# catid/video_stabilizer

Measured on AMD Instinct MI355X. Metric: aligned frames/sec, higher is better.
Workload: dtype u8

## Files before the change

include/vs_amd.h:

```cpp
#ifndef VS_AMD_H
#define VS_AMD_H

#include <stddef.h>
#include <stdint.h>

#ifdef __cplusplus
extern "C" {
#endif

#define VS_OK 0
#define VS_ERR_ARG (-1)
#define VS_ERR_HIP (-2)
#define VS_ERR_UNSUPPORTED (-3)
#define VS_ERR_STATE (-4)
#define VS_ERR_NOMEM (-5)

enum { VS_MEM_HOST = 0, VS_MEM_DEVICE = 1 };
enum { VS_FMT_GRAY8 = 0, VS_FMT_BGR8 = 1, VS_FMT_BGR10 = 2, VS_FMT_BGR12 = 3, VS_FMT_BGR16_FULL = 4 };
int vs_format_bits(int format);
int vs_format_max_value(int format);
enum { VS_WARP_LANCZOS2 = 0, VS_WARP_BILINEAR = 1, VS_WARP_LANCZOS2_FAST = 2, VS_WARP_LANCZOS2_SEP = 3, VS_WARP_BILINEAR_CV = 4 };
enum { VS_BORDER_CLAMP = 0, VS_BORDER_CONSTANT = 1 };
enum {
    VS_SELECT_STL_HOST = 0,
// ... 90 lines not shown
                            void* dst, size_t dst_frame_stride, int dst_stride, int mem, void* stream);
int vs_bgr_image_warp_roi_batch(const void* src, size_t src_frame_stride, int n_frames, int w, int h, int src_stride,
                                int channels, int bits, const vs_transform* t, int mode, int border, int max_value,
                                int roi_x, int roi_y, int roi_w, int roi_h,
                                void* dst, size_t dst_frame_stride, int dst_stride, int mem, void* stream);
int vs_bgr_image_warp_fill_batch(const void* src, size_t src_frame_stride, int n_src, int w, int h, int src_stride,
                                 int channels, int bits, int n_out, int n_cand, const int32_t* cand_frame,
                                 const vs_transform* cand_t, int border, int max_value,
                                 int roi_x, int roi_y, int roi_w, int roi_h,
                                 void* dst, size_t dst_frame_stride, int dst_stride, int mem, void* stream);
typedef struct vs_deblur_params { float sensitivity; float max_ratio; } vs_deblur_params;
void vs_deblur_params_default(vs_deblur_params* p);
int vs_bgr_sharpness_batch(const void* src, size_t src_frame_stride, int n, int w, int h, int src_stride, int format,
                           uint64_t* sharpness, int mem, void* stream);
int vs_bgr_deblur_batch(const void* src, size_t src_frame_stride, int n_src, int w, int h, int src_stride, int format,
                        const uint64_t* sharpness, int n_out, int n_cand, const int32_t* cand_frame, const vs_transform* cand_t,
                        const vs_deblur_params* params ,
                        void* dst, size_t dst_frame_stride, int dst_stride, int mem, void* stream);
int vs_bgr_image_warp_f32(const void* src, int w, int h, int src_stride, int channels, int bits,
                          const vs_transform* t, int mode, int border,
                          float* dst, int dst_stride, int mem, void* stream);
int vs_bgr_to_gray(const void* src, int w, int h, int src_stride, int bits, int shift_to_8,
                   uint8_t* dst, int dst_stride, int mem, void* stream);

typedef struct vs_flow_params {
    double pyr_scale;
    int    levels;
    int    winsize;
    int    iterations;
    int    poly_n;
    double poly_sigma;
    int    flags;
} vs_flow_params;
void vs_flow_params_default(vs_flow_params* p);
typedef struct vs_flow vs_flow;
vs_flow* vs_flow_create(const vs_flow_params* params , int device);
void     vs_flow_destroy(vs_flow* f);
int vs_flow_compute(vs_flow* f, const uint8_t* prev, const uint8_t* next, int w, int h, int stride, int mem, float* flow,
                    int flow_stride);
int vs_flow_jitter(vs_flow* f, const void* frames, size_t frame_stride, int n, int w, int h, int stride, int format, int mem,
                   float* pair_medians, double* median);

int vs_test_fail_alloc(int k);

int vs_debug_bounds_check(void);
int vs_debug_bounds_selftest(void);

int vs_calib_copy12(const void* src_dev, void* dst_dev, size_t bytes, void* stream);
int vs_shader_clock_probe(void* stream, double* shader_mhz);

typedef struct vs_aligner vs_aligner;
typedef struct vs_align_info {
    int32_t status;
    int32_t fail_reason;
    int32_t fail_level;
    int32_t levels;
    int32_t iterations[16];
    double  condition[16];
    double  phase_dx, phase_dy, phase_response;
    int32_t selected_x[16], selected_y[16];
    vs_transform level_transform[16];
} vs_align_info;

vs_aligner* vs_aligner_create(const vs_aligner_params* params , int device);
void vs_aligner_destroy(vs_aligner* a);
int  vs_aligner_set_select_mode(vs_aligner* a, int select_mode);
int  vs_aligner_get_select_mode(const vs_aligner* a);
enum { VS_BATCH_EXCLUSIVE = 0, VS_BATCH_SHARED = 1 };
int  vs_aligner_set_batch_mode(vs_aligner* a, int batch_mode);
int  vs_aligner_reset(vs_aligner* a);
void* vs_aligner_stream(const vs_aligner* a);
int   vs_aligner_wait_stream(vs_aligner* a, void* producer_stream);
int  vs_aligner_align_next(vs_aligner* a, const void* frame, int w, int h, int stride, int format, int mem,
                           const vs_aligner_params* params, vs_transform* out);
int  vs_aligner_align_batch(vs_aligner* a, const void* frames, size_t frame_stride, int n,
                            int w, int h, int stride, int format, int mem,
                            const vs_aligner_params* params, vs_transform* out, int32_t* status);
int  vs_aligner_align_clips(vs_aligner* a, const void* frames, size_t frame_stride, int n_clips, int frames_per_clip,
                            int w, int h, int stride, int format, int mem,
                            const vs_aligner_params* params, vs_transform* out, int32_t* status);
int  vs_aligner_get_info(const vs_aligner* a, int i, vs_align_info* info);
int  vs_aligner_level_dims(const vs_aligner* a, int level, int* w, int* h, int* tiles_x, int* tiles_y, int* tile_size);
int  vs_aligner_read_level_image(const vs_aligner* a, int i, int level, uint8_t* out);
int  vs_aligner_read_level_argmax(const vs_aligner* a, int i, int level, int set, uint16_t* out);
int  vs_aligner_read_level_jacobian(const vs_aligner* a, int i, int level, int set, float* out);

enum {
    VS_STAGE_INGEST = 0,
    VS_STAGE_PYR_DOWN = 1,
    VS_STAGE_KEYFRAME = 2,
    VS_STAGE_WARPDIFF = 3,
    VS_STAGE_SELECT = 4,
    VS_STAGE_GATHER = 5,
    VS_STAGE_GN = 6,
    VS_STAGE_PHASE = 7,
    VS_STAGE_COUNT = 8
};
typedef struct vs_stage_timings {
    double ms[VS_STAGE_COUNT];
    int64_t launches[VS_STAGE_COUNT];
    int64_t frames;
    int64_t gn_iterations;
} vs_stage_timings;
int  vs_aligner_enable_timing(vs_aligner* a, int enable);
int  vs_aligner_get_timings(vs_aligner* a, vs_stage_timings* out);

typedef struct vs_stabilizer vs_stabilizer;
vs_stabilizer* vs_stabilizer_create(const vs_stabilizer_params* params , int device);
void vs_stabilizer_destroy(vs_stabilizer* s);
int  vs_stabilizer_process(vs_stabilizer* s, const void* frame, int w, int h, int stride, int format, int mem,
                           void* out, int* out_w, int* out_h);
int  vs_stabilizer_process_batch(vs_stabilizer* s, const void* frames, size_t frame_stride, int n, int w, int h, int stride,
                                 int format, int mem, void* out, size_t out_frame_stride, int32_t* has_output,
                                 int* out_w, int* out_h);
int  vs_stabilizer_process_clips(vs_stabilizer* s, const void* frames, size_t frame_stride, int n_clips, int frames_per_clip,
                                 int w, int h, int stride, int format, int mem, void* out, size_t out_frame_stride,
                                 int32_t* has_output, int* out_w, int* out_h);
int  vs_stabilizer_reset(vs_stabilizer* s);
void* vs_stabilizer_stream(const vs_stabilizer* s);
int   vs_stabilizer_wait_stream(vs_stabilizer* s, void* producer_stream);
int   vs_stabilizer_set_select_mode(vs_stabilizer* s, int mode);
int   vs_stabilizer_get_select_mode(const vs_stabilizer* s);
int   vs_stabilizer_set_border_fill(vs_stabilizer* s, int ahead);
int   vs_stabilizer_get_border_fill(const vs_stabilizer* s);
int   vs_stabilizer_set_deblur(vs_stabilizer* s, int ahead, const vs_deblur_params* params);
int   vs_stabilizer_get_deblur(const vs_stabilizer* s);
void vs_stabilizer_state(const vs_stabilizer* s, vs_transform* last_meas, vs_transform* accum, int* last_success);

#ifdef __cplusplus
}
#endif
#endif
```

video_stabilizer_amd/capi.py:

```python
import ctypes as C
import os

import numpy as np

_HERE = os.path.dirname(os.path.abspath(__file__))
LIB_PATH = os.environ.get("VS_AMD_LIB", os.path.join(_HERE, "libvs_amd.so"))

MEM_HOST, MEM_DEVICE = 0, 1
FMT_GRAY8, FMT_BGR8 = 0, 1
FMT_BGR10, FMT_BGR12, FMT_BGR16_FULL = 2, 3, 4
WARP_LANCZOS2, WARP_BILINEAR, WARP_LANCZOS2_FAST, WARP_LANCZOS2_SEP, WARP_BILINEAR_CV = 0, 1, 2, 3, 4
BORDER_CLAMP, BORDER_CONSTANT = 0, 1
SELECT_STL_HOST, SELECT_DEVICE, SELECT_STABLE = 0, 1, 2
BATCH_EXCLUSIVE, BATCH_SHARED = 0, 1
ABI_VERSION = 5


class Transform(C.Structure):
    _fields_ = [("A", C.c_double), ("B", C.c_double), ("TX", C.c_double), ("TY", C.c_double)]

    def tup(self):
        return (self.A, self.B, self.TX, self.TY)

    @staticmethod
# ... 55 lines not shown

SIGNATURES = {
    "vs_last_error": (C.c_char_p, []),
    "vs_version": (C.c_char_p, []),
    "vs_abi_version": (_i32, []),
    "vs_sizeof_align_info": (_sz, []),
    "vs_test_fail_alloc": (_i32, [_i32]),
    "vs_debug_bounds_check": (_i32, []),
    "vs_debug_bounds_selftest": (_i32, []),
    "vs_device_count": (_i32, []),
    "vs_shader_clock_probe": (_i32, [C.c_void_p, C.POINTER(C.c_double)]),
    "vs_stream_retire": (_i32, [_vp]),
    "vs_format_bits": (_i32, [_i32]),
    "vs_format_max_value": (_i32, [_i32]),
    "vs_aligner_stream": (_vp, [_vp]),
    "vs_aligner_wait_stream": (_i32, [_vp, _vp]),
    "vs_stabilizer_stream": (_vp, [_vp]),
    "vs_stabilizer_wait_stream": (_i32, [_vp, _vp]),
    "vs_aligner_params_default": (None, [C.POINTER(AlignerParams)]),
    "vs_stabilizer_params_default": (None, [C.POINTER(StabilizerParams)]),
    "vs_transform_inverse": (Transform, [_TP]),
    "vs_transform_compose": (Transform, [_TP, _TP]),
    "vs_transform_warp": (Point, [_TP, Point]),
    "vs_transform_warp_center": (Point, [_TP, Point, _f64, _f64]),
    "vs_transform_max_corner_displacement": (_f64, [_TP, _f64, _f64]),
    "vs_tile_size": (_i32, [_i32, _i32]),
    "vs_ul_params_sparse": (None, [_TP, _i32, _i32, _vp]),
    "vs_ul_params_warp": (None, [_TP, _i32, _i32, _vp]),
    "vs_cv_inverse_matrix": (None, [_TP, _i32, _i32, _vp]),
    "vs_smoother_create": (_vp, [_i32, _i32, _f64]),
    "vs_smoother_destroy": (None, [_vp]),
    "vs_smoother_update": (_i32, [_vp, _TP, _TP]),
    "vs_tvl1_smooth": (None, [_vp, _i32, _f64, _i32, _vp]),
    "vs_calib_copy12": (_i32, [_vp, _vp, _sz, _vp]),
    "vs_pyr_down": (_i32, [_vp, _i32, _i32, _i32, _vp, _i32, _i32, _i32, _i32, _vp]),
    "vs_grad_xy": (_i32, [_vp, _i32, _i32, _i32, _vp, _vp, _i32, _vp]),
    "vs_grad_argmax": (_i32, [_vp, _vp, _i32, _i32, _i32, _vp, _vp, _i32, _vp]),
    "vs_sparse_jac": (_i32, [_vp, _vp, _i32, _i32, _vp, _vp, _i32, _i32, _vp, _vp, _i32, _vp]),
    "vs_keyframe_fused": (_i32, [_vp, _i32, _i32, _i32, _i32, _vp, _vp, _vp, _vp, _i32, _vp]),
    "vs_sparse_warpdiff": (_i32, [_vp, _vp, _i32, _i32, _i32, _vp, _i32, _i32, _f32, _f32, _f32, _f32, _vp, _i32, _vp]),
    "vs_sparse_ica": (_i32, [_vp, _vp, _i32, _i32, _i32, _vp, _i32, _vp, _i32, _vp, _vp, _f32, _f32, _f32, _f32, _vp, _i32, _vp]),
    "vs_select_smallest": (_i32, [_vp, _i32, _i32, _i32, _f32, _vp, _vp, _i32, _vp]),
    "vs_select_smallest_stable": (_i32, [_vp, _i32, _i32, _i32, _f32, _vp, _i32, _vp]),
    "vs_phase_correlate": (_i32, [_vp, _vp, _i32, _i32, _i32, _i32, _vp, _vp, _vp]),
    "vs_optimal_dft_size": (_i32, [_i32]),
    "vs_image_warp": (_i32, [_vp, _i32, _i32, _i32, _f32, _f32, _f32, _f32, _vp, _i32, _i32, _i32, _vp]),
    "vs_bgr_image_warp": (_i32, [_vp, _i32, _i32, _i32, _i32, _i32, _TP, _i32, _i32, _i32, _vp, _i32, _i32, _vp]),
    "vs_bgr_image_warp_batch": (_i32, [_vp, _sz, _i32, _i32, _i32, _i32, _i32, _i32, _TP, _i32, _i32, _i32, _vp, _sz, _i32, _i32, _vp]),
    "vs_bgr_image_warp_roi_batch": (_i32, [_vp, _sz, _i32, _i32, _i32, _i32, _i32, _i32, _TP, _i32, _i32, _i32,
                                           _i32, _i32, _i32, _i32, _vp, _sz, _i32, _i32, _vp]),
    "vs_bgr_image_warp_fill_batch": (_i32, [_vp, _sz, _i32, _i32, _i32, _i32, _i32, _i32, _i32, _i32, C.POINTER(C.c_int32), _TP, _i32, _i32,
                                            _i32, _i32, _i32, _i32, _vp, _sz, _i32, _i32, _vp]),
    "vs_deblur_params_default": (None, [C.POINTER(DeblurParams)]),
    "vs_bgr_sharpness_batch": (_i32, [_vp, _sz, _i32, _i32, _i32, _i32, _i32, _vp, _i32, _vp]),
    "vs_bgr_deblur_batch": (_i32, [_vp, _sz, _i32, _i32, _i32, _i32, _i32, _vp, _i32, _i32, C.POINTER(C.c_int32), _TP, C.POINTER(DeblurParams),
                                   _vp, _sz, _i32, _i32, _vp]),
    "vs_bgr_image_warp_f32": (_i32, [_vp, _i32, _i32, _i32, _i32, _i32, _TP, _i32, _i32, _vp, _i32, _i32, _vp]),
    "vs_bgr_to_gray": (_i32, [_vp, _i32, _i32, _i32, _i32, _i32, _vp, _i32, _i32, _vp]),
    "vs_flow_params_default": (None, [C.POINTER(FlowParams)]),
    "vs_flow_create": (_vp, [C.POINTER(FlowParams), _i32]),
    "vs_flow_destroy": (None, [_vp]),
    "vs_flow_compute": (_i32, [_vp, _vp, _vp, _i32, _i32, _i32, _i32, _vp, _i32]),
    "vs_flow_jitter": (_i32, [_vp, _vp, _sz, _i32, _i32, _i32, _i32, _i32, _i32, _vp, C.POINTER(C.c_double)]),
    "vs_aligner_create": (_vp, [C.POINTER(AlignerParams), _i32]),
    "vs_aligner_destroy": (None, [_vp]),
    "vs_aligner_set_select_mode": (_i32, [_vp, _i32]),
    "vs_stabilizer_set_select_mode": (_i32, [_vp, _i32]),
    "vs_aligner_get_select_mode": (_i32, [_vp]),
    "vs_stabilizer_get_select_mode": (_i32, [_vp]),
    "vs_stabilizer_set_border_fill": (_i32, [_vp, _i32]),
    "vs_stabilizer_get_border_fill": (_i32, [_vp]),
    "vs_stabilizer_set_deblur": (_i32, [_vp, _i32, C.POINTER(DeblurParams)]),
    "vs_stabilizer_get_deblur": (_i32, [_vp]),
    "vs_aligner_set_batch_mode": (_i32, [_vp, _i32]),
    "vs_aligner_reset": (_i32, [_vp]),
    "vs_aligner_align_next": (_i32, [_vp, _vp, _i32, _i32, _i32, _i32, _i32, C.POINTER(AlignerParams), _TP]),
    "vs_aligner_align_batch": (_i32, [_vp, _vp, _sz, _i32, _i32, _i32, _i32, _i32, _i32, C.POINTER(AlignerParams), _TP, C.POINTER(C.c_int32)]),
    "vs_aligner_align_clips": (_i32, [_vp, _vp, _sz, _i32, _i32, _i32, _i32, _i32, _i32, _i32, C.POINTER(AlignerParams), _TP, C.POINTER(C.c_int32)]),
    "vs_aligner_enable_timing": (_i32, [_vp, _i32]),
    "vs_aligner_get_timings": (_i32, [_vp, C.POINTER(StageTimings)]),
    "vs_aligner_get_info": (_i32, [_vp, _i32, C.POINTER(AlignInfo)]),
    "vs_aligner_level_dims": (_i32, [_vp, _i32, _IP, _IP, _IP, _IP, _IP]),
    "vs_aligner_read_level_image": (_i32, [_vp, _i32, _i32, _vp]),
    "vs_aligner_read_level_argmax": (_i32, [_vp, _i32, _i32, _i32, _vp]),
    "vs_aligner_read_level_jacobian": (_i32, [_vp, _i32, _i32, _i32, _vp]),
    "vs_stabilizer_create": (_vp, [C.POINTER(StabilizerParams), _i32]),
    "vs_stabilizer_destroy": (None, [_vp]),
    "vs_stabilizer_process": (_i32, [_vp, _vp, _i32, _i32, _i32, _i32, _i32, _vp, _IP, _IP]),
    "vs_stabilizer_process_batch": (_i32, [_vp, _vp, _sz, _i32, _i32, _i32, _i32, _i32, _i32, _vp, _sz, C.POINTER(C.c_int32), _IP, _IP]),
    "vs_stabilizer_process_clips": (_i32, [_vp, _vp, _sz, _i32, _i32, _i32, _i32, _i32, _i32, _i32, _vp, _sz, C.POINTER(C.c_int32), _IP, _IP]),
    "vs_stabilizer_reset": (_i32, [_vp]),
    "vs_stabilizer_state": (None, [_vp, _TP, _TP, _IP]),
}

_lib = None


def lib():
    global _lib
    if _lib is not None:
        return _lib
    if not os.path.exists(LIB_PATH):
        raise VsError("libvs_amd.so is missing (%s): run `python -c 'import __graft_entry__ as g; g.build()'`" % LIB_PATH)
    L = C.CDLL(LIB_PATH)
    partial = os.environ.get("VS_AMD_LIB_PARTIAL") == "1"
    for name, (res, args) in SIGNATURES.items():
        if partial and not hasattr(L, name):
            continue
        fn = getattr(L, name)
        fn.restype = res
        fn.argtypes = args
    if L.vs_abi_version() != ABI_VERSION or L.vs_sizeof_align_info() != C.sizeof(AlignInfo):
        raise VsError("libvs_amd.so has ABI %d (vs_align_info %d bytes); this binding was written for ABI %d (%d bytes)"
                      % (L.vs_abi_version(), L.vs_sizeof_align_info(), ABI_VERSION, C.sizeof(AlignInfo)))
    _lib = L
    return L


def _check(r):
    if r < 0:
        raise VsError("vs_amd error %d: %s" % (r, lib().vs_last_error().decode()))
    return r


def _p(a):
    if isinstance(a, np.ndarray):
        return a.ctypes.data_as(C.c_void_p)
    return C.c_void_p(int(a))


def _c(a, dtype):
    return np.ascontiguousarray(a, dtype=dtype)


def device_count():
    return lib().vs_device_count()


def shader_clock_probe(stream=None):
    mhz = C.c_double(0.0)
    _check(lib().vs_shader_clock_probe(C.c_void_p(stream) if stream else None, C.byref(mhz)))
    return mhz.value


def debug_bounds_check():
    r = lib().vs_debug_bounds_check()
    if r < 0:
        raise VsError("vs_amd error %d: %s" % (r, lib().vs_last_error().decode()))
    return r, (lib().vs_last_error().decode() if r else "")


def test_fail_alloc(k):
    return lib().vs_test_fail_alloc(int(k))


def aligner_params(**kw):
    p = AlignerParams()
    lib().vs_aligner_params_default(C.byref(p))
    for k, v in kw.items():
        setattr(p, k, v)
    return p


def stabilizer_params(**kw):
    p = StabilizerParams()
    lib().vs_stabilizer_params_default(C.byref(p))
# ... 452 lines not shown
        _check(lib().vs_aligner_set_batch_mode(self.h, mode))

    def align_next(self, frame, fmt=None):
        frame = np.ascontiguousarray(frame)
        fmt = _fmt_of(frame.dtype, frame.ndim) if fmt is None else fmt
        hh, ww = frame.shape[:2]
        stride = ww * (1 if fmt == FMT_GRAY8 else 3)
        t = Transform()
        r = _check(lib().vs_aligner_align_next(self.h, _p(frame), ww, hh, stride, fmt, MEM_HOST, C.byref(self.params), C.byref(t)))
        return bool(r), t

    def align_batch(self, frames, fmt=None):
        frames = np.ascontiguousarray(frames)
        n = frames.shape[0]
        fmt = _fmt_of(frames.dtype, frames.ndim - 1) if fmt is None else fmt
        hh, ww = frames.shape[1:3]
        ch = 1 if fmt == FMT_GRAY8 else 3
        out = (Transform * n)()
        status = (C.c_int32 * n)()
        _check(lib().vs_aligner_align_batch(self.h, _p(frames), hh * ww * ch, n, ww, hh, ww * ch, fmt, MEM_HOST,
                                            C.byref(self.params), out, status))
        return list(status), list(out)

    def align_batch_device(self, ptr, n, w, h, fmt, stride=None, frame_stride=None):
        ch = 1 if fmt == FMT_GRAY8 else 3
        stride = stride or w * ch
        frame_stride = frame_stride or h * stride
        out = (Transform * n)()
        status = (C.c_int32 * n)()
        _check(lib().vs_aligner_align_batch(self.h, _p(ptr), frame_stride, n, w, h, stride, fmt, MEM_DEVICE,
                                            C.byref(self.params), out, status))
        return list(status), list(out)

    def align_clips(self, frames, n_clips, mem_ptr=None, w=None, h=None, fmt=None, raw=False):
        if mem_ptr is None:
            frames = np.ascontiguousarray(frames)
            n = frames.shape[0]
            fmt = _fmt_of(frames.dtype, frames.ndim - 1) if fmt is None else fmt
            h, w = frames.shape[1:3]
            ptr, mem = _p(frames), MEM_HOST
        else:
            n, ptr, mem = int(frames), _p(mem_ptr), MEM_DEVICE
        ch = 1 if fmt == FMT_GRAY8 else 3
        out = (Transform * n)()
        status = (C.c_int32 * n)()
        _check(lib().vs_aligner_align_clips(self.h, ptr, h * w * ch, n_clips, n // n_clips, w, h, w * ch, fmt, mem,
                                            C.byref(self.params), out, status))
        if raw:
            return status, out
        return list(status), list(out)

    def reset(self):
        _check(lib().vs_aligner_reset(self.h))

    def enable_timing(self, on=True):
        _check(lib().vs_aligner_enable_timing(self.h, 1 if on else 0))

    def timings(self):
        t = StageTimings()
        _check(lib().vs_aligner_get_timings(self.h, C.byref(t)))
        d = {name: {"ms": t.ms[i], "launches": t.launches[i]} for i, name in enumerate(STAGES)}
        d["frames"] = t.frames
        d["gn_iterations"] = t.gn_iterations
        return d

    def wait_stream(self, stream_handle):
        _check(lib().vs_aligner_wait_stream(self.h, C.c_void_p(stream_handle)))

    def info(self, i=0):
        inf = AlignInfo()
        _check(lib().vs_aligner_get_info(self.h, i, C.byref(inf)))
        return inf

    def level(self, i, level):
        w, h, tx, ty, ts = (C.c_int() for _ in range(5))
        _check(lib().vs_aligner_level_dims(self.h, level, *(C.byref(v) for v in (w, h, tx, ty, ts))))
        w, h, tx, ty, ts = (v.value for v in (w, h, tx, ty, ts))
        d = {"w": w, "h": h, "tx": tx, "ty": ty, "ts": ts}
        img = np.empty((h, w), np.uint8)
        _check(lib().vs_aligner_read_level_image(self.h, i, level, _p(img)))
        d["img"] = img
        return d

    def keyframe_tables(self, i, level):
        w, h, tx, ty, ts = (C.c_int() for _ in range(5))
        _check(lib().vs_aligner_level_dims(self.h, level, *(C.byref(v) for v in (w, h, tx, ty, ts))))
        tx, ty = tx.value, ty.value
        out = {"argmax": [], "jac": []}
        for s in (0, 1):
            am = np.empty((2, ty, tx), np.uint16)
            jc = np.empty((4, ty, tx), np.float32)
            _check(lib().vs_aligner_read_level_argmax(self.h, i, level, s, _p(am)))
            _check(lib().vs_aligner_read_level_jacobian(self.h, i, level, s, _p(jc)))
            out["argmax"].append(am)
            out["jac"].append(jc)
        return out

    def __del__(self):
        if getattr(self, "h", None) and _lib is not None:
            _lib.vs_aligner_destroy(self.h)
            self.h = None


class Stabilizer:

    def __init__(self, device=0, select_mode=None, border_fill=0, deblur=0, deblur_params=None, **params):
        self.params = stabilizer_params(**params)
        self.h = lib().vs_stabilizer_create(C.byref(self.params), device)
        if not self.h:
            raise VsError("vs_stabilizer_create failed: %s" % lib().vs_last_error().decode())
        if select_mode is not None:
            self.set_select_mode(select_mode)
        if border_fill:
            self.set_border_fill(border_fill)
        if deblur:
            self.set_deblur(deblur, deblur_params)

    def set_deblur(self, ahead, params=None):
        _check(lib().vs_stabilizer_set_deblur(self.h, int(ahead), C.byref(params) if params is not None else None))

    def deblur(self):
        return _check(lib().vs_stabilizer_get_deblur(self.h))

    def set_border_fill(self, ahead):
        _check(lib().vs_stabilizer_set_border_fill(self.h, int(ahead)))

    def border_fill(self):
        return _check(lib().vs_stabilizer_get_border_fill(self.h))

    def set_select_mode(self, mode):
        _check(lib().vs_stabilizer_set_select_mode(self.h, mode))

    def select_mode(self):
        return _check(lib().vs_stabilizer_get_select_mode(self.h))

    def process(self, frame, fmt=None):
        frame = np.ascontiguousarray(frame)
        fmt = _fmt_of(frame.dtype, frame.ndim) if fmt is None else fmt
        hh, ww = frame.shape[:2]
        c = max(self.params.crop_pixels, 0)
        out = np.empty((hh - 2 * c, ww - 2 * c, 3), frame.dtype)
        ow, oh = C.c_int(), C.c_int()
        r = _check(lib().vs_stabilizer_process(self.h, _p(frame), ww, hh, ww * 3, fmt, MEM_HOST, _p(out), C.byref(ow), C.byref(oh)))
        return out if r == 1 else None

    def reset(self):
        _check(lib().vs_stabilizer_reset(self.h))

    def wait_stream(self, stream_handle):
        _check(lib().vs_stabilizer_wait_stream(self.h, C.c_void_p(stream_handle)))

    def process_batch(self, frames, out=None, fmt=None):
        frames = np.ascontiguousarray(frames)
        n, hh, ww = frames.shape[:3]
        fmt = _fmt_of(frames.dtype, 3) if fmt is None else fmt
        c = max(self.params.crop_pixels, 0)
        if out is None:
            out = np.zeros((n, hh - 2 * c, ww - 2 * c, 3), frames.dtype)
        assert out.shape == (n, hh - 2 * c, ww - 2 * c, 3) and out.dtype == frames.dtype and out.flags.c_contiguous
        has = (C.c_int32 * n)()
        ow, oh = C.c_int(), C.c_int()
        _check(lib().vs_stabilizer_process_batch(self.h, _p(frames), hh * ww * 3, n, ww, hh, ww * 3, fmt, MEM_HOST, _p(out),
                                                 out[0].size, has, C.byref(ow), C.byref(oh)))
        return out, list(has)

    def process_batch_device(self, ptr, n, w, h, fmt, out_ptr):
# ... 38 lines not shown
```

video_stabilizer_amd/csrc/vs_align_kernels.inc:

```
#define VS_LDS_AS __attribute__((address_space(3)))
constexpr int kVF = kGnVirt / kGnThreads;
constexpr int kVWaves = kGnVirt / 64;
constexpr int kRWaves = kGnThreads / 64;
static_assert(kGnVirt % kGnThreads == 0 && (kVF == 1 || (kVF == 2 && kRWaves == 4)), "virtual-thread layouts: 1:1, or 256 threads for 512");
struct GnShared {
    double red[2][kVWaves * 10];
    double hinv[17];
    double c0[8];
    double c1[8];
    double T[4];
    int flag;
    double Tp[2][4];
    int seq;
    int ctl[2];
};

__device__ __forceinline__ void first_pass_terms(int r, int nsel, const float jf[4], float residual, double (&a8)[8]) {
    const float rx = r < nsel ? residual : 0.0f, ry = r < nsel ? 0.0f : residual;
#pragma unroll
    for (int c = 0; c < 4; c++) {
        a8[c] += (double)(jf[c] * rx);
        a8[4 + c] += (double)(jf[c] * ry);
    }
}
// ... 900 lines not shown
    const int w_lo = min(wave * per, nt), w_hi = min(w_lo + per, nt);
    auto below = [&](unsigned long long m) -> uint32_t {
        return __builtin_amdgcn_mbcnt_hi((uint32_t)(m >> 32), __builtin_amdgcn_mbcnt_lo((uint32_t)m, 0u));
    };
    unsigned long long mine = 0ull;
    for (int s = 0; s < nsets; s++) {
        VS_SPAN(key_t*, a, VS_SPAN_RAW(s ? a1 : a0), nt, 117);
        const uint32_t D = s ? D1 : D0;
        uint32_t less = 0u, eq = 0u;
        for (int i0 = w_lo; i0 < w_hi; i0 += 64 * kP) {
            uint32_t v[kP];
#pragma unroll
            for (int u = 0; u < kP; u++) v[u] = a[min(i0 + 64 * u + lane, nt - 1)];
#pragma unroll
            for (int u = 0; u < kP; u++) {
                const uint32_t d = (i0 + 64 * u + lane < w_hi) ? (v[u] >> 16) : 0xffffffffu;
                less += (uint32_t)__popcll(__ballot(d < D));
                eq += (uint32_t)__popcll(__ballot(d == D));
            }
        }
        mine |= ((unsigned long long)(less | (eq << 16))) << (32 * s);
    }
    if (lane == 0) ss.wsum[wave] = mine;
    __syncthreads();
    unsigned long long before = 0ull;
    for (int w = 0; w < wave; w++) before += ss.wsum[w];
    for (int s = 0; s < nsets; s++) {
        VS_SPAN(key_t*, a, VS_SPAN_RAW(s ? a1 : a0), nt, 117);
        VS_SPAN(out_t*, o, VS_SPAN_RAW(s ? o1 : o0), nt, 118);
        const uint32_t D = s ? D1 : D0, R = s ? R1 : R0;
        uint32_t less = (uint32_t)(before >> (32 * s)) & 0xffffu, eq = (uint32_t)(before >> (32 * s + 16)) & 0xffffu;
        for (int i0 = w_lo; i0 < w_hi; i0 += 64 * kP) {
            uint32_t v[kP];
#pragma unroll
            for (int u = 0; u < kP; u++) v[u] = a[min(i0 + 64 * u + lane, nt - 1)];
#pragma unroll
            for (int u = 0; u < kP; u++) {
                const int i = i0 + 64 * u + lane;
                const uint32_t d = i < w_hi ? (v[u] >> 16) : 0xffffffffu;
                const unsigned long long ml = __ballot(d < D), me = __ballot(d == D);
                const uint32_t my_less = less + below(ml), my_eq = eq + below(me);
                if (d < D || (d == D && my_eq < R)) o[my_less + min(my_eq, R)] = (uint16_t)i;
                less += (uint32_t)__popcll(ml);
                eq += (uint32_t)__popcll(me);
            }
        }
    }
    __syncthreads();
}


__global__ VS_GN_FUSED_BOUNDS __attribute__((unused)) void vs_k_select(const uint16_t* __restrict__ wd, int nt, int nsel,
                                                          int32_t* __restrict__ out_idx, int32_t* __restrict__ status, int rule) {
    extern __shared__ __attribute__((aligned(16))) uint8_t dyn[];
    __shared__ SelShared ss;
    __shared__ StableShared sts;
    uint32_t* a = (uint32_t*)dyn;
    uint16_t* posR = (uint16_t*)(a + nt);
    wd += (size_t)blockIdx.x * nt;
    out_idx += (size_t)blockIdx.x * nt;
    for (int i = threadIdx.x; i < nt; i += kGnThreads) a[i] = ((uint32_t)wd[i] << 16) | (uint32_t)i;
    __syncthreads();
    if (rule) {
        stable_select<true>(a, posR, a, posR, 1, nt, nsel, sts);
        for (int i = threadIdx.x; i < nsel; i += kGnThreads) out_idx[i] = (int32_t)posR[i];
        if (status != nullptr && threadIdx.x == 0) status[blockIdx.x] = 0;
        return;
    }
    const int r = introselect_block(a, posR, ss, nt, nsel);
    for (int i = threadIdx.x; i < nsel; i += kGnThreads) out_idx[i] = (int32_t)(a[i] & 0xffffu);
    if (threadIdx.x == 0) status[blockIdx.x] = r;
}


__global__ VS_GN_FUSED_BOUNDS void vs_k_align_pairs(PairState* __restrict__ states,
                                                               const PairDesc* __restrict__ descs,
                                                               const uint8_t* __restrict__ pyr, size_t pyr_frame,
                                                               const uint16_t* __restrict__ lm_tab, size_t lm_frame,
                                                               const float* __restrict__ jac_tab, size_t jac_frame,
                                                               uint8_t* __restrict__ recs, size_t recs_pair,
                                                               int nt_cap, int dyn_bytes, FusedLevels fl, GnParams gp,
                                                               int group, uint8_t* __restrict__ coop, int epoch,
                                                               float* __restrict__ wv_all, PairDescPack dpack, int direct,
                                                               uint8_t* __restrict__ selbuf, size_t selbuf_pair) {
    extern __shared__ __attribute__((aligned(16))) uint8_t dyn[];
    __shared__ SelShared ss2[2];
    __shared__ GnShared sh;
    __shared__ int s_coop[2];
    __shared__ __attribute__((aligned(16))) uint32_t sel_tail[(kWaveRange + 1) + (kWaveRange + 2) / 2 + 32];
    static_assert(sizeof(StableShared) <= sizeof(sel_tail), "VS_SELECT_STABLE keeps its histograms in the tail block (unused in that mode)");
    uint32_t* a = (uint32_t*)dyn;
    uint16_t* posR = (uint16_t*)(a + nt_cap);
    int p = blockIdx.x / group;
    const int g = blockIdx.x % group;
    if (group == 1) {
        const int n = (int)gridDim.x, x = (int)blockIdx.x & 7;
        p = (n >> 3) * x + min(x, n & 7) + ((int)blockIdx.x >> 3);
    }
    CoopCtrl* const cc = group > 1 ? (CoopCtrl*)(coop + (size_t)p * coop_pair_bytes(nt_cap)) : nullptr;
    uint32_t* const gkeys = group > 1 ? (uint32_t*)((uint8_t*)cc + kCoopCtrlBytes) : nullptr;
    float* const wv = wv_all + (size_t)p * 2 * nt_cap;
    float* const gvals = group > 1 ? (float*)(gkeys + 2 * (size_t)nt_cap) : nullptr;
    float* const gtpx = group > 1 ? gvals + 2 * (size_t)nt_cap : nullptr;
    float* const wt = wv + (size_t)gridDim.x / group * 2 * nt_cap;
    auto ld_sc1 = [](const int* f) { return __hip_atomic_load(f, __ATOMIC_RELAXED, __HIP_MEMORY_SCOPE_AGENT); };
    auto st_sc1 = [](int* f, int v) { __hip_atomic_store(f, v, __ATOMIC_RELAXED, __HIP_MEMORY_SCOPE_AGENT); };
    auto ldd_sc1 = [](const double* f) { return __hip_atomic_load(f, __ATOMIC_RELAXED, __HIP_MEMORY_SCOPE_AGENT); };
    auto std_sc1 = [](double* f, double v) { __hip_atomic_store(f, v, __ATOMIC_RELAXED, __HIP_MEMORY_SCOPE_AGENT); };
    auto flag_wait = [&](const int* f) -> bool {
        for (int it = 0; it < (1 << 18); it++) {
            if (ld_sc1(f) == epoch) return true;
            if (g > 0 && ld_sc1(&cc->abort) == epoch) return false;
            __builtin_amdgcn_s_sleep(4);
        }
        return false;
    };
    PairState& st = states[p];
    const PairDesc d = direct ? dpack.d[p] : descs[p];
    double T[4] = {0.0, 0.0, 0.0, 0.0};
    if (!direct) { T[0] = st.T[0]; T[1] = st.T[1]; T[2] = st.T[2]; T[3] = st.T[3]; }
    int fail = 0, fail_level = 0;
    if (g > 0 && threadIdx.x == 0) st_sc1(&cc->arrived[g], epoch);
    for (int l = fl.levels - 1; l >= 0 && !fail; l--) {
        const int w = fl.w[l], h = fl.h[l], nt = fl.nt[l], nsel = fl.nsel[l];
        const bool share = group > 1 && nt >= kCoopMinTiles;
        if (g > 0 && !share) continue;
        int my_slice = 0, nslices = 1;
        if (g > 0) {
            if (threadIdx.x == 0) s_coop[0] = flag_wait(&cc->lv[l].t_ready) ? 1 : 0;
            __syncthreads();
            if (!s_coop[0]) return;
            const int sl_ = ld_sc1(&cc->lv[l].assign[g]), ns_ = ld_sc1(&cc->lv[l].nslices);
            const double t0_ = ldd_sc1(&cc->lv[l].T[0]), t1_ = ldd_sc1(&cc->lv[l].T[1]), t2_ = ldd_sc1(&cc->lv[l].T[2]), t3_ = ldd_sc1(&cc->lv[l].T[3]);
            my_slice = sl_; nslices = ns_;
            T[0] = t0_; T[1] = t1_; T[2] = t2_; T[3] = t3_;
            __syncthreads();
            if (my_slice < 0) continue;
        }
        const uint8_t* tmpl = pyr + (size_t)d.tmpl_slot * pyr_frame + fl.img_off[l];
        const uint8_t* key = pyr + (size_t)d.key_slot * pyr_frame + fl.img_off[l];
        const PointRecs rc = pair_recs(recs, recs_pair, p, nt_cap);
        float P[4];
        ul_params_sparse(T, w, h, P);
        const float A1 = 1.0f + P[0];
        const uint16_t* lm0 = lm_tab + (size_t)d.key_slot * lm_frame + fl.lm_off[l];
        const float* jac0 = jac_tab + (size_t)d.key_slot * jac_frame + fl.jac_off[l];
        auto stage_image = [&]() {
            const uint32_t* src = (const uint32_t*)key;
            uint32_t* dst = (uint32_t*)dyn;
            typedef uint32_t u32x4 __attribute__((ext_vector_type(4)));
            const VS_GLOBAL_AS u32x4* __restrict__ s4 = (const VS_GLOBAL_AS u32x4*)key;
            VS_LDS_AS u32x4* __restrict__ d4 = (VS_LDS_AS u32x4*)(uintptr_t)(unsigned)(uintptr_t)dyn;
            const int n4 = (w * h) / 16;
            for (int i = threadIdx.x; i < n4; i += 4 * kGnThreads) {
                u32x4 v[4];
#pragma unroll
                for (int u = 0; u < 4; u++) v[u] = s4[min(i + u * kGnThreads, n4 - 1)];
#pragma unroll
                for (int u = 0; u < 4; u++) if (i + u * kGnThreads < n4) d4[i + u * kGnThreads] = v[u];
            }
            for (int i = n4 * 4 + threadIdx.x; i < (w * h) / 4; i += kGnThreads) dst[i] = src[i];
            VS_BOUNDS_CHECK((w * h) / 4 + 1, dyn_bytes / 4, 120);
            if (threadIdx.x < 2) dst[(w * h) / 4 + threadIdx.x] = 0u;
        };
        const int img_bytes = (w * h + 8 + 15) & ~15;
        const bool img_fits = l == fl.levels - 1 && w * h + 8 <= dyn_bytes && (w * h & 3) == 0;
        const bool img_first = img_fits && g == 0 && img_bytes + 12 * nt <= dyn_bytes && nt <= 32 * (kGnThreads / 2);
        const bool sel_global = selbuf != nullptr && 6 * nt > dyn_bytes;
        if (img_first) {
            stage_image();
            a = (uint32_t*)(dyn + img_bytes);
            __syncthreads();
        } else if (sel_global) {
            a = (uint32_t*)(selbuf + (size_t)p * selbuf_pair);
            posR = (uint16_t*)(a + nt_cap);
        } else {
            a = (uint32_t*)dyn;
            if (selbuf != nullptr) posR = (uint16_t*)(a + nt);
        }
        const vs_lbytes lkey_img = (vs_lbytes)(uintptr_t)(unsigned)(uintptr_t)dyn;
        const int row_pts = 2 * fl.tx[l];
        auto point_tile = [&](int i, int& set, int& t) {
            const int j = i / row_pts, q = i - j * row_pts;
            set = q >= fl.tx[l] ? 1 : 0;
            t = j * fl.tx[l] + q - set * fl.tx[l];
        };
        constexpr int kWdFlight = 1;
        auto warpdiff_fill = [&](auto gkey, uint32_t* dst, const uint16_t* __restrict__ lmb, int count, bool both, int voff) {
            const vs_gbytes gtmpl = (vs_gbytes)tmpl;
            const VS_GLOBAL_AS uint32_t* __restrict__ gxy = (const VS_GLOBAL_AS uint32_t*)lmb;
            uint32_t lx[kWdFlight], ly[kWdFlight];
            auto load_lm = [&](int b) {
#pragma unroll
                for (int u = 0; u < kWdFlight; u++) {
                    const int i = min(b + u * kGnThreads, count - 1);
                    int set = 0, t = i;
                    if (both) point_tile(i, set, t);
                    const uint32_t xy = gxy[set * nt + t];
                    lx[u] = xy & 0xffffu; ly[u] = xy >> 16;
                }
            };
            int base = threadIdx.x;
            if (base < count) load_lm(base);
            while (base < count) {
                LanczosFetch f[kWdFlight];
                uint32_t tp[kWdFlight];
#pragma unroll
                for (int u = 0; u < kWdFlight; u++) {
                    const int tile_x = min((int)lx[u], w - 1), tile_y = min((int)ly[u], h - 1);
                    const float ox = (float)tile_x, oy = (float)tile_y;
                    const float Wx = A1 * ox - P[1] * oy + P[2];
                    const float Wy = P[1] * ox + A1 * oy + P[3];
                    f[u] = lanczos_fetch(gkey, w, h, w, Wx, Wy);
                    tp[u] = gtmpl[(size_t)tile_y * w + tile_x];
                }
                const int nb = base + kWdFlight * kGnThreads;
                if (nb < count) load_lm(nb);
#pragma unroll
                for (int u = 0; u < kWdFlight; u++) {
                    const int i = base + u * kGnThreads;
                    const float v = lanczos_finish(f[u], w);
                    float diff = fabsf(v - (float)tp[u]);
                    diff = fminf(fmaxf(diff, 0.0f), 65535.0f);
                    if (i < count) {
                        int set = 0, t = i;
                        if (both) point_tile(i, set, t);
                        const int o = set * nt + t;
                        VS_BOUNDS_CHECK(o, both ? 2 * nt : nt, 121);
                        VS_BOUNDS_CHECK(voff + o, 2 * nt_cap, 122);
                        dst[o] = ((uint32_t)(uint16_t)diff << 16) | (uint32_t)t;
                        wv[voff + o] = v;
                        wt[voff + o] = (float)tp[u];
                    }
                }
                base = nb;
            }
        };
        auto warpdiff_slice = [&](uint32_t* __restrict__ dst, uint32_t* stage, int i0_all, int i1_all) {
            const vs_gbytes gkey = (vs_gbytes)key, gtmpl = (vs_gbytes)tmpl;
            const VS_GLOBAL_AS uint32_t* __restrict__ gxy = (const VS_GLOBAL_AS uint32_t*)lm0;
            lds_u32* __restrict__ stg = (lds_u32*)stage;
            const int cap = (dyn_bytes / 12) & ~63;
            for (int i0 = i0_all; i0 < i1_all; i0 += cap) {
            const int i1 = min(i0 + cap, i1_all), n = i1 - i0;
            for (int base = threadIdx.x; base < n; base += 4 * kGnThreads) {
                uint32_t lx[4], ly[4];
#pragma unroll
                for (int u = 0; u < 4; u++) {
                    const int i = i0 + min(base + u * kGnThreads, n - 1);
                    const uint32_t xy = gxy[i];
                    lx[u] = xy & 0xffffu; ly[u] = xy >> 16;
                }
                LanczosFetch f[4];
                uint32_t tp[4];
                float vv[4];
#pragma unroll
                for (int u = 0; u < 4; u++) {
                    const int tile_x = min((int)lx[u], w - 1), tile_y = min((int)ly[u], h - 1);
                    const float ox = (float)tile_x, oy = (float)tile_y;
                    f[u] = lanczos_fetch(gkey, w, h, w, A1 * ox - P[1] * oy + P[2], P[1] * ox + A1 * oy + P[3]);
                    tp[u] = gtmpl[(size_t)tile_y * w + tile_x];
                }
#pragma unroll
                for (int u = 0; u < 4; u++) {
                    const int q = base + u * kGnThreads, i = i0 + q;
                    vv[u] = lanczos_finish(f[u], w);
                    float diff = fabsf(vv[u] - (float)tp[u]);
                    diff = fminf(fmaxf(diff, 0.0f), 65535.0f);
                    if (q < n) {
                        VS_BOUNDS_CHECK(2 * n + q, dyn_bytes / 4, 123);
                        stg[q] = ((uint32_t)(uint16_t)diff << 16) | (uint32_t)(i - (i >= nt ? nt : 0));
                        stg[n + q] = __float_as_uint(vv[u]);
                        stg[2 * n + q] = __float_as_uint((float)tp[u]);
                    }
                }
            }
            __syncthreads();
            typedef uint32_t u32x4 __attribute__((ext_vector_type(4)));
            for (int q = 4 * (int)threadIdx.x; q < n; q += 4 * kGnThreads) {
                if (q + 4 <= n) {
                    const u32x4 v = {stg[q], stg[q + 1], stg[q + 2], stg[q + 3]}, x = {stg[n + q], stg[n + q + 1], stg[n + q + 2], stg[n + q + 3]},
                                y = {stg[2 * n + q], stg[2 * n + q + 1], stg[2 * n + q + 2], stg[2 * n + q + 3]};
                    asm volatile("global_store_dwordx4 %0, %1, off sc1\n\ts_nop 1" :: "v"(dst + i0 + q), "v"(v) : "memory");
                    asm volatile("global_store_dwordx4 %0, %1, off sc1\n\ts_nop 1" :: "v"(gvals + i0 + q), "v"(x) : "memory");
                    asm volatile("global_store_dwordx4 %0, %1, off sc1\n\ts_nop 1" :: "v"(gtpx + i0 + q), "v"(y) : "memory");
                } else {
                    for (int u = 0; q + u < n; u++) {
                        st_sc1((int*)dst + i0 + q + u, (int)stg[q + u]); st_sc1((int*)gvals + i0 + q + u, (int)stg[n + q + u]);
                        st_sc1((int*)gtpx + i0 + q + u, (int)stg[2 * n + q + u]);
                    }
                }
            }
            __syncthreads();
            }
            asm volatile("s_waitcnt vmcnt(0)" ::: "memory");
        };
        constexpr int kGaFlight = 4;
        double hacc[10] = {0, 0, 0, 0, 0, 0, 0, 0, 0, 0};
        double fa8[8] = {0, 0, 0, 0, 0, 0, 0, 0};
        auto gather_fill = [&](const uint32_t* sel, const uint16_t* sel16, int count, bool both, const uint16_t* __restrict__ lmb,
                               const float* __restrict__ jacb, int slot0, int voff) {
            const lds_u16* __restrict__ lsel16 = (const lds_u16*)sel16;
            const VS_GLOBAL_AS uint16_t* __restrict__ gsel16 = (const VS_GLOBAL_AS uint16_t*)sel16;
            typedef float f32x4g __attribute__((ext_vector_type(4)));
            const VS_GLOBAL_AS uint32_t* __restrict__ gxy = (const VS_GLOBAL_AS uint32_t*)lmb;
            const VS_GLOBAL_AS f32x4g* __restrict__ gj = (const VS_GLOBAL_AS f32x4g*)jacb;
            const lds_u32* __restrict__ lsel = (const lds_u32*)sel;
            const glb_u32* __restrict__ gsel = (const glb_u32*)sel;
            int first = (int)threadIdx.x - slot0 % kGnThreads;
            if (first < 0) first += kGnThreads;
            for (int base = first; base < count; base += kGaFlight * kGnThreads) {
                uint32_t px[kGaFlight], py[kGaFlight];
                float jv[kGaFlight][4], sv[kGaFlight], tp[kGaFlight];
#pragma unroll
                for (int u = 0; u < kGaFlight; u++) {
                    const int j = min(base + u * kGnThreads, count - 1);
                    const int set = (both && j >= nsel) ? 1 : 0;
                    VS_BOUNDS_CHECK(j + set * (nt - nsel), both ? 2 * nt : nt, 124);
                    const int t = sel16 != nullptr ? (int)(sel_global ? gsel16[j + set * (nt - nsel)] : lsel16[j + set * (nt - nsel)])
                                                   : (int)((sel_global ? gsel[j + set * (nt - nsel)] : lsel[j + set * (nt - nsel)]) & 0xffffu);
                    VS_BOUNDS_CHECK(t, nt, 125);
                    VS_BOUNDS_CHECK(voff + set * nt + t, 2 * nt_cap, 126);
                    const uint32_t xy = gxy[set * nt + VS_DEBUG_CLAMP(t, nt)];
                    px[u] = xy & 0xffffu; py[u] = xy >> 16;
                    const f32x4g jq = gj[set * nt + VS_DEBUG_CLAMP(t, nt)];
                    jv[u][0] = jq.x; jv[u][1] = jq.y; jv[u][2] = jq.z; jv[u][3] = jq.w;
                    sv[u] = wv[voff + set * nt + t];
                    tp[u] = wt[voff + set * nt + t];
                }
#pragma unroll
                for (int u = 0; u < kGaFlight; u++) {
                    const int j = base + u * kGnThreads;
                    if (j < count) {
                        const int slot = slot0 + j;
                        VS_BOUNDS_CHECK(slot, 2 * nt_cap, 127);
                        rc.xy[slot] = px[u] | (py[u] << 16);
                        rc.tv[slot] = tp[u];
                        const float r0 = tp[u] - sv[u];
                        rc.r0[slot] = r0;
                        rc.j[slot] = make_float4(jv[u][0], jv[u][1], jv[u][2], jv[u][3]);
                        if (kVF == 1) {
                            first_pass_terms(slot, nsel, jv[u], r0, fa8);
                            const double jd[4] = {(double)jv[u][0], (double)jv[u][1], (double)jv[u][2], (double)jv[u][3]};
                            int k = 0;
// ... 154 lines not shown
```

video_stabilizer_amd/csrc/vs_engine.hip:

```cpp
#include "vs_internal.hpp"
#include "vs_kernels.hpp"
#include "vs_phase.hpp"
#include "vs_device.hpp"

#include <algorithm>
#include <atomic>
#include <chrono>
#include <mutex>
#include <cmath>
#include <cstring>
#include <deque>
#include <thread>
#include <cstdlib>
#include <future>
#include <string>
#include <vector>

using vsi::set_error;
using namespace vsd;

#define VS_TRY(expr) do { int _r = (expr); if (_r < 0) return _r; } while (0)
#define VS_ARG(cond) do { if (!(cond)) return set_error(VS_ERR_ARG, "bad argument: %s (%s)", #cond, __func__); } while (0)

namespace {

constexpr int kMaxLevels = 16;
constexpr int kSelectCap = 26000;

struct LevelDims {
    int w, h, ts, tx, ty, nt, nsel;
    size_t img_off;
    size_t lm_off;
    size_t jac_off;
};

struct PairState {
    double T[4];
    int32_t status;
    int32_t fail_reason;
    int32_t fail_level;
    int32_t pad;
    int32_t iterations[kMaxLevels];
    double condition[kMaxLevels];
    double level_T[kMaxLevels][4];
};

struct PairDesc {
    int32_t tmpl_slot;
    int32_t key_slot;
};

constexpr int kDirectMaxPairs = 16;
struct PairDescPack { PairDesc d[kDirectMaxPairs]; };

struct GnParams {
    double threshold, max_displacement;
    int max_iters;
    int pipeline;
    int stall_helpers;
    int sel_depth_cap;
    int sel_stable;
};

__global__ void vs_k_phase_apply(PairState* __restrict__ states, const vsp::Result* __restrict__ res,
                                 const uint8_t* __restrict__ negate, int n_pairs, double threshold, float scale) {
    const int q = blockIdx.x * blockDim.x + threadIdx.x;
    if (q >= n_pairs) return;
    const vsp::Result r = res[q];
    if (r.response > threshold) {
        double tx = r.dx * scale, ty = r.dy * scale;
        if (negate[q]) { tx = -tx; ty = -ty; }
        states[q].T[2] = tx;
        states[q].T[3] = ty;
    }
}

__global__ __launch_bounds__(256) void vs_k_warpdiff_batch(const PairState* __restrict__ states,
                                                           const PairDesc* __restrict__ descs,
                                                           const uint8_t* __restrict__ pyr, size_t pyr_frame,
                                                           size_t img_off, int w, int h,
                                                           const uint16_t* __restrict__ lm_tab, size_t lm_frame,
                                                           size_t lm_off, int nt, uint16_t* __restrict__ wd,
                                                           float* __restrict__ wv, size_t wd_pair) {
    const int p = blockIdx.y, set = blockIdx.z;
    const PairState& st = states[p];
    if (st.status != 1) return;
    const int i = blockIdx.x * 256 + threadIdx.x;
    if (i >= nt) return;
    const PairDesc d = descs[p];
    const uint8_t* tmpl = pyr + (size_t)d.tmpl_slot * pyr_frame + img_off;
    const uint8_t* key = pyr + (size_t)d.key_slot * pyr_frame + img_off;
    const uint16_t* lm = lm_tab + (size_t)d.key_slot * lm_frame + lm_off + (size_t)set * 2 * nt;
    double T[4] = {st.T[0], st.T[1], st.T[2], st.T[3]};
    float P[4];
    ul_params_sparse(T, w, h, P);
    const uint32_t xy = ((const uint32_t*)lm)[i];
    int tile_x = min((int)(xy & 0xffffu), w - 1), tile_y = min((int)(xy >> 16), h - 1);
    float ox = (float)tile_x, oy = (float)tile_y;
    float Wx = (1.0f + P[0]) * ox - P[1] * oy + P[2];
    float Wy = P[1] * ox + (1.0f + P[0]) * oy + P[3];
    float v = lanczos_sample_u8(key, w, h, w, Wx, Wy);
    float diff = fabsf(v - (float)tmpl[(size_t)tile_y * w + tile_x]);
    diff = fminf(fmaxf(diff, 0.0f), 65535.0f);
    wd[(size_t)p * wd_pair + (size_t)set * nt + i] = (uint16_t)diff;
    wv[(size_t)p * wd_pair + (size_t)set * nt + i] = v;
}

template <typename T>
__device__ __forceinline__ T* uniform_ptr(T* p) {
    const unsigned long long v = (unsigned long long)p;
    const unsigned lo = __builtin_amdgcn_readfirstlane((unsigned)v), hi = __builtin_amdgcn_readfirstlane((unsigned)(v >> 32));
    return (T*)(((unsigned long long)hi << 32) | lo);
}

struct PointRecs {
    uint32_t* xy;
    float* tv;
    float4* j;
    float* r0;
};
__device__ __forceinline__ PointRecs pair_recs(uint8_t* recs, size_t recs_pair, int p, int nt_cap) {
    uint8_t* base = recs + (size_t)p * recs_pair;
    PointRecs r;
    r.j = (float4*)base;
    r.xy = (uint32_t*)(base + (size_t)2 * nt_cap * 16);
    r.tv = (float*)(base + (size_t)2 * nt_cap * 20);
    r.r0 = (float*)(base + (size_t)2 * nt_cap * 24);
    return r;
}
__device__ __forceinline__ void write_rec(const PointRecs& rc, int slot, const uint16_t* __restrict__ lm,
                                          const float* __restrict__ jac, int nt, int t, const uint8_t* __restrict__ tmpl,
                                          int w, int h, const float* __restrict__ wv_set) {
    const uint32_t xy = ((const uint32_t*)lm)[t];
    const int px = (int)(xy & 0xffffu), py = (int)(xy >> 16);
    rc.xy[slot] = xy;
    const float tv = (float)tmpl[(size_t)min(py, h - 1) * w + min(px, w - 1)];
    rc.tv[slot] = tv;
    rc.r0[slot] = tv - wv_set[t];
    rc.j[slot] = ((const float4*)jac)[t];
}

__global__ __launch_bounds__(256) void vs_k_gather_selected(const PairState* __restrict__ states,
                                                            const PairDesc* __restrict__ descs,
                                                            const uint8_t* __restrict__ pyr, size_t pyr_frame,
                                                            size_t img_off, int w, int h,
                                                            const uint16_t* __restrict__ lm_tab, size_t lm_frame,
                                                            size_t lm_off, const float* __restrict__ jac_tab,
                                                            size_t jac_frame, size_t jac_off, int nt, int nsel,
                                                            const int32_t* __restrict__ idx, size_t idx_pair,
                                                            const float* __restrict__ wv,
                                                            uint8_t* __restrict__ recs, size_t recs_pair, int nt_cap) {
    const int p = blockIdx.y, set = blockIdx.z;
    if (states[p].status != 1) return;
    const int j = blockIdx.x * 256 + threadIdx.x;
    if (j >= nsel) return;
    const PairDesc d = descs[p];
    const uint16_t* lm = lm_tab + (size_t)d.key_slot * lm_frame + lm_off + (size_t)set * 2 * nt;
    const float* jac = jac_tab + (size_t)d.key_slot * jac_frame + jac_off + (size_t)set * 4 * nt;
    const uint8_t* tmpl = pyr + (size_t)d.tmpl_slot * pyr_frame + img_off;
    const int t = idx[(size_t)p * idx_pair + (size_t)set * nt + j];
    write_rec(pair_recs(recs, recs_pair, p, nt_cap), set * nsel + j, lm, jac, nt, t, tmpl, w, h, wv + (size_t)p * idx_pair + (size_t)set * nt);
}

constexpr int kMaxDevices = 64;
constexpr int kCoopGroup = 16;
constexpr int kCoopMaxGroup = 16;
constexpr int kCoopMaxPairs = 128;
constexpr int kChipCUs = 256;
constexpr int kCoopMinTiles = 4096;
struct CoopLevel {
    int t_ready, nslices, pad[2];
    int assign[kCoopMaxGroup];
    int wd_done[kCoopMaxGroup];
    double T[4];
};
struct CoopCtrl {
    int arrived[kCoopMaxGroup];
    int abort;
    int pad[15];
    CoopLevel lv[kMaxLevels];
};
constexpr size_t kCoopCtrlBytes = (sizeof(CoopCtrl) + 255) & ~(size_t)255;
__host__ __device__ inline size_t coop_pair_bytes(int nt_cap) { return kCoopCtrlBytes + (((size_t)nt_cap * 24 + 255) & ~(size_t)255); }

struct FusedLevels {
    int levels;
    int w[kMaxLevels], h[kMaxLevels], nt[kMaxLevels], nsel[kMaxLevels], tx[kMaxLevels];
    unsigned long long img_off[kMaxLevels], lm_off[kMaxLevels], jac_off[kMaxLevels];
};

namespace nt1024 {
constexpr int kGnThreads = 1024, kGnVirt = 1024;
#define VS_GN_FUSED_BOUNDS __launch_bounds__(kGnThreads)
#include "vs_align_kernels.inc"
#undef VS_GN_FUSED_BOUNDS
}
namespace nt512 {
constexpr int kGnThreads = 512, kGnVirt = 512;
#define VS_GN_FUSED_BOUNDS __launch_bounds__(kGnThreads)
#include "vs_align_kernels.inc"
#undef VS_GN_FUSED_BOUNDS
}
namespace nt256v {
constexpr int kGnThreads = 256, kGnVirt = 512;
#define VS_GN_FUSED_BOUNDS __launch_bounds__(kGnThreads, 4)
#include "vs_align_kernels.inc"
#undef VS_GN_FUSED_BOUNDS
}
constexpr int kCoResidentMaxTiles = 128 * 256;
constexpr int kSharedMinPairs = 32;
constexpr size_t kCoResidentDynMax = 32 * 1024;
constexpr int kSmallWgTiles = 26000;
constexpr int kPipelineMaxPairs = 128;

}

VS_BOUNDS_TU(vs_bounds_fetch_engine)

static size_t ingest_chunk_bytes() {
    const char* e = getenv("VS_INGEST_CHUNK_BYTES");
    const long long v = e ? atoll(e) : 0;
    return v > 0 ? (size_t)v : (size_t)192 << 20;
}
#define kIngestBytes ingest_chunk_bytes()

template <typename F, typename... A>
static std::future<hipError_t> run_async(F&& fn, A&&... args) {
    try {
        return std::async(std::launch::async, fn, args...);
    } catch (...) {
        return std::async(std::launch::deferred, fn, args...);
    }
}

struct vs_aligner {
    int device = 0;
    hipStream_t stream = nullptr;
    vs_aligner_params params;
    int select_mode = VS_SELECT_DEVICE;
    int batch_mode = VS_BATCH_EXCLUSIVE;
    int cu_count = kChipCUs;
    bool coop_ok = true;

    int W = -1, H = -1, fmt = -1;
    int levels = 0;
    LevelDims L[kMaxLevels];
    long long seq = 0;
    int clip_len = 0;
    size_t pyr_frame = 0, lm_frame = 0, jac_frame = 0;
    int nt_max = 0;

    int cap = 0;
    uint8_t* pyr = nullptr;
    uint16_t* lm = nullptr;
    float* jac = nullptr;
    PairState* states = nullptr;
    PairDesc* descs = nullptr;
    uint16_t* wd = nullptr;
    float* wv = nullptr;
    int32_t* idx = nullptr;
    uint8_t* recs = nullptr;
    uint8_t* coop = nullptr;
    uint8_t* selbuf = nullptr; size_t selbuf_bytes = 0;
    int coop_epoch = 0;
    void* stage = nullptr; size_t stage_bytes = 0;
    void* ingest[2] = {nullptr, nullptr}; size_t ingest_bytes = 0;
    hipStream_t copy_stream = nullptr;
    vsp::Context phase;
    int phase_cap = 0;
    float2* pspec = nullptr;
    float2* pG = nullptr;
    float* psurf = nullptr;
    vsp::Pair* ppairs = nullptr;
    uint8_t* pneg = nullptr;
    vsp::Result* pres = nullptr;
    std::vector<vsp::Result> h_pres;
    uint16_t* h_wd = nullptr;
    int32_t* h_idx = nullptr;
    PairState* h_states = nullptr;
    PairDesc* h_descs = nullptr;

    std::vector<vs_align_info> info;
    int last_n = 0;

    bool timing = false;
    vs_stage_timings tm{};
    struct Span { int stage; hipEvent_t a, b; };
    std::vector<Span> spans;
    std::vector<hipEvent_t> event_pool;
    hipEvent_t get_event() {
        if (!event_pool.empty()) { hipEvent_t e = event_pool.back(); event_pool.pop_back(); return e; }
        hipEvent_t e; (void)hipEventCreate(&e); return e;
    }
    void t_begin(int stage) {
        if (!timing) return;
        Span sp{stage, get_event(), get_event()};
        (void)hipEventRecord(sp.a, stream);
        spans.push_back(sp);
    }
    void t_end(int launches) {
        if (!timing) return;
        (void)hipEventRecord(spans.back().b, stream);
        tm.launches[spans.back().stage] += launches;
    }
    void t_collect() {
        for (Span& sp : spans) {
            float ms = 0.f;
            if (hipEventElapsedTime(&ms, sp.a, sp.b) == hipSuccess) tm.ms[sp.stage] += ms;
            event_pool.push_back(sp.a); event_pool.push_back(sp.b);
        }
        spans.clear();
    }

    ~vs_aligner() {
        release();
        for (hipEvent_t e : event_pool) (void)hipEventDestroy(e);
        if (copy_stream) (void)hipStreamDestroy(copy_stream);
        if (stream) { (void)vsi::retire_stream(stream); (void)hipStreamDestroy(stream); }
    }
    void release();
    int configure(int w, int h, int format, const vs_aligner_params& p);
    int ensure_capacity(int n);
    int ensure_phase();
    void release_phase();
    struct Chunk {
        bool open = false;
        int n = 0, n_pairs = 0, epoch = 0;
        long long seq0 = 0;
        vs_aligner_params p;
        vs_transform* out = nullptr; int32_t* status = nullptr; vs_align_info* infos = nullptr;
        std::vector<int> pair_frame;
        bool direct = false, use_host = false;
        GnParams gp{};
    } ck;
    int chunk_begin(const void* frames, size_t frame_stride, int n, int stride, int mem, const vs_aligner_params& p,
                    vs_transform* out, int32_t* status, vs_align_info* infos);
    int chunk_end();
    int run_chunk(const void* frames, size_t frame_stride, int n, int stride, int mem, const vs_aligner_params& p,
                  vs_transform* out, int32_t* status, vs_align_info* infos) {
        VS_TRY(chunk_begin(frames, frame_stride, n, stride, mem, p, out, status, infos));
        return chunk_end();
    }
    int select_host(int n_pairs, const LevelDims& l);
    bool started = false, started_clips = false;
    int started_n = 0, started_result = 0;
    int32_t* started_status = nullptr;
};

void vs_aligner::release_phase() {
    void* d[] = {pspec, pG, psurf, ppairs, pneg, pres};
    for (void* p : d) if (p) (void)hipFree(p);
    pspec = nullptr; pG = nullptr; psurf = nullptr; ppairs = nullptr; pneg = nullptr; pres = nullptr;
    phase_cap = 0;
    phase.destroy();
}

int vs_aligner::ensure_phase() {
    const LevelDims& pl = L[2];
    if (phase.w != pl.w || phase.h != pl.h) {
        release_phase();
        const hipError_t pe = phase.configure(pl.w, pl.h, stream);
        if (pe == hipErrorInvalidValue)
            return set_error(VS_ERR_UNSUPPORTED, "phase_correlate: level 2 is %dx%d, padded extent over %d", pl.w, pl.h, vsp::kMaxLine);
        VS_HIP(pe);
    }
    if (phase_cap >= cap) return VS_OK;
    void* d[] = {pspec, pG, psurf, ppairs, pneg, pres};
    for (void* p : d) if (p) (void)hipFree(p);
    pspec = nullptr; pG = nullptr; psurf = nullptr; ppairs = nullptr; pneg = nullptr; pres = nullptr; phase_cap = 0;
    VS_HIP(vsi::dev_alloc((void**)&pspec, ((size_t)cap + 1) * phase.spec_frame() * sizeof(float2)));
    VS_HIP(vsi::dev_alloc((void**)&pG, (size_t)cap * phase.spec_frame() * sizeof(float2)));
    VS_HIP(vsi::dev_alloc((void**)&psurf, (size_t)cap * phase.surface_elems() * sizeof(float)));
    VS_HIP(vsi::dev_alloc((void**)&ppairs, (size_t)cap * sizeof(vsp::Pair)));
    VS_HIP(vsi::dev_alloc((void**)&pneg, (size_t)cap));
    VS_HIP(vsi::dev_alloc((void**)&pres, (size_t)cap * sizeof(vsp::Result)));
    phase_cap = cap;
    return VS_OK;
}

void vs_aligner::release() {
    release_phase();
    void* d[] = {pyr, lm, jac, states, descs, wd, wv, idx, recs, coop, stage, ingest[0], ingest[1], selbuf};
    for (void* p : d) if (p) (void)hipFree(p);
    selbuf = nullptr; selbuf_bytes = 0;
    ingest[0] = ingest[1] = nullptr; ingest_bytes = 0;
    void* hp[] = {h_wd, h_idx, h_states, h_descs};
    for (void* p : hp) if (p) (void)hipHostFree(p);
    pyr = nullptr; lm = nullptr; jac = nullptr; states = nullptr; descs = nullptr; wd = nullptr; wv = nullptr; idx = nullptr;
    recs = nullptr; coop = nullptr; stage = nullptr; stage_bytes = 0; h_wd = nullptr; h_idx = nullptr; h_states = nullptr; h_descs = nullptr;
    cap = 0;
}

int vs_aligner::configure(int w, int h, int format, const vs_aligner_params& p) {
    int lv = 0, ww = w, hh = h;
    do { lv++; ww /= 2; hh /= 2; } while (ww >= p.pyramid_min_width && hh >= p.pyramid_min_height);
    if (lv < 3 || lv > kMaxLevels)
        return set_error(VS_ERR_UNSUPPORTED, "%dx%d with pyramid_min %dx%d gives %d pyramid levels; 3..%d supported", w, h,
                         p.pyramid_min_width, p.pyramid_min_height, lv, kMaxLevels);
    if (w > 65535 || h > 65535) return set_error(VS_ERR_UNSUPPORTED, "frame larger than 65535 (u16 keypoints)");
    ww = w; hh = h;
    for (int i = 0; i < lv; i++) {
        if (i > 0) { ww /= 2; hh /= 2; }
        const int ts = vs_tile_size(ww, hh);
        if (ww < 4 || hh < 4 || (ww / ts) * (hh / ts) < 1)
            return set_error(VS_ERR_UNSUPPORTED, "pyramid level %d is %dx%d: levels below 4x4 are not supported", i, ww, hh);
    }
    release();
    W = w; H = h; fmt = format; levels = lv; seq = 0;
    size_t img = 0, lmo = 0, jo = 0;
    nt_max = 0;
    ww = w; hh = h;
    for (int i = 0; i < lv; i++) {
        if (i > 0) { ww /= 2; hh /= 2; }
        LevelDims& l = L[i];
        l.w = ww; l.h = hh;
        l.ts = vs_tile_size(ww, hh);
        l.tx = ww / l.ts; l.ty = hh / l.ts; l.nt = l.tx * l.ty;
        l.nsel = (int)static_cast<size_t>((size_t)l.nt * p.smallest_fraction);
        l.img_off = img; img += ((size_t)ww * hh + 255) & ~(size_t)255;
        l.lm_off = lmo; lmo += (size_t)l.nt * 4;
        l.jac_off = jo; jo += (size_t)l.nt * 8;
        nt_max = std::max(nt_max, l.nt);
    }
    pyr_frame = img; lm_frame = (lmo + 63) & ~(size_t)63; jac_frame = (jo + 63) & ~(size_t)63;
    return VS_OK;
}

int vs_aligner::ensure_capacity(int n) {
    if (n <= cap) return VS_OK;
    const int newcap = n;
    const size_t slots = (size_t)newcap + 1;
    const size_t coop_bytes = std::min(newcap, kCoopMaxPairs) * coop_pair_bytes(nt_max);
    struct NewSet {
        void* dev[10] = {};
        void* pinned[4] = {};
        ~NewSet() {
            for (void* q : dev) if (q) (void)hipFree(q);
            for (void* q : pinned) if (q) (void)hipHostFree(q);
        }
    } ns;
    enum { D_PYR, D_LM, D_JAC, D_STATES, D_DESCS, D_WD, D_IDX, D_WV, D_RECS, D_COOP };
    const size_t dev_bytes[10] = {
        slots * pyr_frame, slots * lm_frame * 2, slots * jac_frame * 4, sizeof(PairState) * newcap, sizeof(PairDesc) * newcap,
        (size_t)newcap * 2 * nt_max * sizeof(uint16_t), (size_t)newcap * 2 * nt_max * sizeof(int32_t),
        (size_t)newcap * 2 * nt_max * sizeof(float) * 2,
        (size_t)newcap * 2 * nt_max * 28, coop_bytes};
    const size_t pinned_bytes[4] = {(size_t)newcap * 2 * nt_max * sizeof(uint16_t), (size_t)newcap * 2 * nt_max * sizeof(int32_t),
                                    sizeof(PairState) * newcap, sizeof(PairDesc) * newcap};
    for (int i = 0; i < 10; i++) VS_HIP(vsi::dev_alloc(&ns.dev[i], dev_bytes[i]));
    for (int i = 0; i < 4; i++) VS_HIP(vsi::pinned_alloc(&ns.pinned[i], pinned_bytes[i]));
    VS_HIP(hipMemsetAsync(ns.dev[D_COOP], 0, coop_bytes, stream));
    const bool carry = pyr && seq > 0;
    if (carry) {
        VS_HIP(hipMemcpyAsync(ns.dev[D_PYR], pyr + (size_t)last_n * pyr_frame, pyr_frame, hipMemcpyDeviceToDevice, stream));
        VS_HIP(hipMemcpyAsync(ns.dev[D_LM], lm + (size_t)last_n * lm_frame, lm_frame * 2, hipMemcpyDeviceToDevice, stream));
        VS_HIP(hipMemcpyAsync(ns.dev[D_JAC], jac + (size_t)last_n * jac_frame, jac_frame * 4, hipMemcpyDeviceToDevice, stream));
    }
    VS_HIP(hipStreamSynchronize(stream));
    void** dev_members[10] = {(void**)&pyr, (void**)&lm, (void**)&jac, (void**)&states, (void**)&descs, (void**)&wd, (void**)&idx,
                              (void**)&wv, (void**)&recs, (void**)&coop};
    void** pinned_members[4] = {(void**)&h_wd, (void**)&h_idx, (void**)&h_states, (void**)&h_descs};
    for (int i = 0; i < 10; i++) std::swap(*dev_members[i], ns.dev[i]);
    for (int i = 0; i < 4; i++) std::swap(*pinned_members[i], ns.pinned[i]);
    if (carry) last_n = 0;
    coop_epoch = 0;
    cap = newcap;
    return VS_OK;
}

int vs_aligner::select_host(int n_pairs, const LevelDims& l) {
    struct DeltaPixel { uint16_t abs_delta, tile_x, tile_y; };
    const int nt = l.nt, nsel = l.nsel, tx = l.tx;
    const size_t wd_pair = (size_t)2 * nt_max;
    auto work = [&](int begin, int end) {
        std::vector<DeltaPixel> v;
        for (int job = begin; job < end; job++) {
            const int p = job >> 1, set = job & 1;
            if (h_states[p].status != 1) continue;
            const uint16_t* src = h_wd + (size_t)p * wd_pair + (size_t)set * nt;
            if (select_mode == VS_SELECT_STABLE) {
                std::vector<uint64_t> key((size_t)nt);
                for (int i = 0; i < nt; i++) key[i] = ((uint64_t)src[i] << 32) | (uint32_t)i;
                std::vector<uint64_t> sorted(key);
                int32_t* dst = h_idx + (size_t)p * wd_pair + (size_t)set * nt;
                if (nsel > 0) {
                    std::nth_element(sorted.begin(), sorted.begin() + (nsel - 1), sorted.end());
                    const uint64_t cut = sorted[nsel - 1];
                    int m = 0;
                    for (int i = 0; i < nt; i++) if (key[i] <= cut) dst[m++] = i;
                }
                continue;
            }
            v.clear();
            v.reserve(nt);
            for (int j = 0; j < l.ty; j++)
                for (int k = 0; k < tx; k++)
                    v.push_back(DeltaPixel{src[(size_t)j * tx + k], (uint16_t)k, (uint16_t)j});
            std::nth_element(v.begin(), v.begin() + nsel, v.end(),
                             [](const DeltaPixel& a, const DeltaPixel& b) { return a.abs_delta < b.abs_delta; });
            int32_t* dst = h_idx + (size_t)p * wd_pair + (size_t)set * nt;
            for (int j = 0; j < nsel; j++) dst[j] = (int32_t)v[j].tile_y * tx + v[j].tile_x;
        }
    };
    const int jobs = n_pairs * 2;
    int nthreads = (int)std::min<unsigned>(std::max(1u, std::thread::hardware_concurrency()), 16u);
    nthreads = std::min(nthreads, std::max(1, jobs / 8));
    if (nthreads <= 1) {
        work(0, jobs);
    } else {
        std::vector<std::thread> th;
        const int per = (jobs + nthreads - 1) / nthreads;
        for (int t = 0; t < nthreads; t++) {
            int b = t * per, e = std::min(jobs, b + per);
            if (b < e) th.emplace_back(work, b, e);
        }
        for (auto& t : th) t.join();
    }
    return VS_OK;
}

int vs_aligner::chunk_begin(const void* frames, size_t frame_stride, int n, int stride, int mem,
                            const vs_aligner_params& p, vs_transform* out, int32_t* status, vs_align_info* infos) {
    hipStream_t s = stream;
    if (ck.open) return set_error(VS_ERR_ARG, "a chunk is already in flight on this handle");
    ck.n = n; ck.p = p; ck.out = out; ck.status = status; ck.infos = infos; ck.seq0 = seq;
    ck.n_pairs = 0; ck.direct = false; ck.use_host = false; ck.pair_frame.clear();
    const int ch = fmt == VS_FMT_GRAY8 ? 1 : 3;
    const int fbits = vs_format_bits(fmt);
    const size_t esz = fbits > 8 ? 2 : 1;

    if (seq > 0 && last_n != 0) {
        VS_HIP(hipMemcpyAsync(pyr, pyr + (size_t)last_n * pyr_frame, pyr_frame, hipMemcpyDeviceToDevice, s));
        VS_HIP(hipMemcpyAsync(lm, lm + (size_t)last_n * lm_frame, lm_frame * 2, hipMemcpyDeviceToDevice, s));
        VS_HIP(hipMemcpyAsync(jac, jac + (size_t)last_n * jac_frame, jac_frame * 4, hipMemcpyDeviceToDevice, s));
    }

    const void* dframes = frames;
    t_begin(VS_STAGE_INGEST);
    if (mem == VS_MEM_HOST) {
        const size_t bytes = ((size_t)(n - 1) * frame_stride + (size_t)(H - 1) * stride + (size_t)W * ch) * esz;
        if (bytes > stage_bytes) {
            if (stage) (void)hipFree(stage);
            stage = nullptr; stage_bytes = 0;
            VS_HIP(vsi::dev_alloc(&stage, bytes));
            stage_bytes = bytes;
        }
        VS_HIP(hipMemcpyAsync(stage, frames, bytes, hipMemcpyHostToDevice, s));
        dframes = stage;
    }
    uint8_t* slot1 = pyr + pyr_frame;
    if (fmt == VS_FMT_GRAY8) {
        for (int i = 0; i < n; i++)
            VS_HIP(hipMemcpy2DAsync(slot1 + (size_t)i * pyr_frame, W, (const uint8_t*)dframes + (size_t)i * frame_stride,
                                    stride, W, H, hipMemcpyDeviceToDevice, s));
    } else {
        VS_HIP(vsk::ingest_pyr(dframes, W, H, stride, fbits > 8 ? 16 : 8, fbits - 8, slot1,
                               slot1 + L[1].img_off, n, frame_stride, pyr_frame, s));
    }
    t_end(1);
    t_begin(VS_STAGE_PYR_DOWN);
    for (int l = (fmt == VS_FMT_GRAY8 ? 1 : 2); l < levels; l++)
        VS_HIP(vsk::pyr_down(slot1 + L[l - 1].img_off, L[l - 1].w, L[l - 1].h, L[l - 1].w, slot1 + L[l].img_off, L[l].w,
                             L[l].h, L[l].w, n, pyr_frame, pyr_frame, s));
    t_end(levels - (fmt == VS_FMT_GRAY8 ? 1 : 2));

    if (p.phase_correlate) {
        VS_TRY(ensure_phase());
        t_begin(VS_STAGE_PHASE);
        const int first = (seq > 0 && clip_len == 0) ? 0 : 1;
        VS_HIP(phase.spectra(pyr + (size_t)first * pyr_frame + L[2].img_off, pyr_frame, L[2].w, n + 1 - first,
                             pspec + (size_t)first * phase.spec_frame(), s));
        t_end(2);
    }

    auto gidx = [&](int i) -> long long { return clip_len > 0 ? (long long)(i % clip_len) : seq + i; };
    {
        std::vector<std::pair<int, int>> runs;
        if (clip_len > 0 && (clip_len & 1)) for (int c0 = 0; c0 < n; c0 += clip_len) runs.emplace_back(c0, std::min(clip_len, n - c0));
        else runs.emplace_back(0, n);
        bool any = false;
        int kf_launches = 0;
        for (auto& r : runs) {
            const int first_odd = r.first + ((gidx(r.first) & 1) ? 0 : 1);
            const int n_odd = first_odd < r.first + r.second ? (r.first + r.second - first_odd + 1) / 2 : 0;
            if (n_odd <= 0) continue;
            if (!any) { t_begin(VS_STAGE_KEYFRAME); any = true; }
            const size_t so = (size_t)(first_odd + 1);
            vsk::KeyframeLevels KL{};
            KL.n = levels;
            for (int l = 0; l < levels; l++)
                KL.lv[l] = vsk::KeyframeLevel{L[l].w, L[l].h, L[l].ts, L[l].tx, L[l].ty, 0, 0, L[l].img_off, L[l].lm_off, L[l].jac_off};
            if (vsk::keyframe_levels_supported(KL)) {
                VS_HIP(vsk::keyframe_levels(pyr + so * pyr_frame, lm + so * lm_frame, jac + so * jac_frame, KL, n_odd, 2 * pyr_frame,
                                            2 * lm_frame, 2 * jac_frame, s));
                kf_launches += 1;
            } else {
                for (int l = 0; l < levels; l++) {
                    uint16_t* lmx = lm + so * lm_frame + L[l].lm_off;
                    float* jx = jac + so * jac_frame + L[l].jac_off;
                    VS_HIP(vsk::keyframe(pyr + so * pyr_frame + L[l].img_off, L[l].w, L[l].h, L[l].w, L[l].ts, lmx,
                                         lmx + 2 * (size_t)L[l].nt, jx, jx + 4 * (size_t)L[l].nt, n_odd, 2 * pyr_frame,
                                         2 * lm_frame, 2 * jac_frame, s, true));
                }
                kf_launches += levels;
            }
        }
        if (any) t_end(kf_launches);
    }

    std::vector<int>& pair_frame = ck.pair_frame;
    pair_frame.reserve(n);
    for (int i = 0; i < n; i++) {
        memset(&infos[i], 0, sizeof(vs_align_info));
        infos[i].levels = levels;
        out[i] = vs_transform{0, 0, 0, 0};
        status[i] = 0;
        if (gidx(i) >= 1) pair_frame.push_back(i);
        else infos[i].fail_reason = 1;
    }
    const int n_pairs = (int)pair_frame.size();
    ck.n_pairs = n_pairs;
    if (n_pairs > 0) {
        PairDesc* hd = h_descs;
        for (int q = 0; q < n_pairs; q++) {
            const int i = pair_frame[q];
            const int cur = i + 1, prev = i;
            if (gidx(i) & 1) { hd[q].key_slot = cur; hd[q].tmpl_slot = prev; }
            else { hd[q].key_slot = prev; hd[q].tmpl_slot = cur; }
        }
        for (int q = 0; q < n_pairs; q++) {
            memset(&h_states[q], 0, sizeof(PairState));
            h_states[q].status = 1;
        }
        const bool direct = n_pairs <= kDirectMaxPairs && !p.phase_correlate && select_mode != VS_SELECT_STL_HOST && nt_max <= kSelectCap;
        ck.direct = direct;
        if (!direct) {
            VS_HIP(hipMemcpyAsync(descs, hd, sizeof(PairDesc) * n_pairs, hipMemcpyHostToDevice, s));
            VS_HIP(hipMemcpyAsync(states, h_states, sizeof(PairState) * n_pairs, hipMemcpyHostToDevice, s));
        }
        std::vector<vsp::Pair> hp;
        std::vector<uint8_t> hneg;
        const float phase_scale = (1 << 2) / float(1 << levels);
        auto apply_phase = [&]() -> int {
            hipLaunchKernelGGL(vs_k_phase_apply, dim3((n_pairs + 255) / 256), dim3(256), 0, s, states, pres, pneg, n_pairs,
                               p.phase_correlate_threshold, phase_scale);
            VS_HIP(hipGetLastError());
            return VS_OK;
        };
        if (p.phase_correlate) {
            hp.resize(n_pairs); hneg.resize(n_pairs);
            for (int q = 0; q < n_pairs; q++) {
                const int i = pair_frame[q];
                hp[q] = vsp::Pair{i, i + 1};
                hneg[q] = (gidx(i) & 1) ? 1 : 0;
            }
            VS_HIP(hipMemcpyAsync(ppairs, hp.data(), sizeof(vsp::Pair) * n_pairs, hipMemcpyHostToDevice, s));
            VS_HIP(hipMemcpyAsync(pneg, hneg.data(), (size_t)n_pairs, hipMemcpyHostToDevice, s));
            t_begin(VS_STAGE_PHASE);
            VS_HIP(phase.correlate(pspec, ppairs, n_pairs, pG, psurf, pres, s));
            VS_TRY(apply_phase());
            t_end(4);
            h_pres.resize(n_pairs);
            VS_HIP(hipMemcpyAsync(h_pres.data(), pres, sizeof(vsp::Result) * n_pairs, hipMemcpyDeviceToHost, s));
        }
        if (p.phase_correlate) VS_HIP(hipStreamSynchronize(s));

        const size_t recs_pair = (size_t)2 * nt_max * 28;
        static const int pipe_env = []() { const char* e = getenv("VS_GN_PIPELINE"); return e ? atoi(e) : -1; }();
        const int pipeline = pipe_env >= 0 ? pipe_env : (n_pairs <= kPipelineMaxPairs ? 1 : 0);
        static const int stall_env = []() { const char* e = getenv("VS_GN_STALL_HELPERS"); return e ? atoi(e) : 0; }();
        static const int depth_env = []() { const char* e = getenv("VS_GN_SELECT_DEPTH"); return e ? atoi(e) : 0; }();
        GnParams gp{p.threshold, p.max_displacement, p.max_iters, pipeline, stall_env, depth_env, select_mode == VS_SELECT_STABLE ? 1 : 0};
        ck.gp = gp;
        const bool use_host = select_mode == VS_SELECT_STL_HOST || nt_max > kSelectCap;
        ck.use_host = use_host;
        if (!use_host) {
            FusedLevels fl;
            fl.levels = levels;
            for (int l = 0; l < levels; l++) {
                fl.w[l] = L[l].w; fl.h[l] = L[l].h; fl.nt[l] = L[l].nt; fl.nsel[l] = L[l].nsel; fl.tx[l] = L[l].tx;
                fl.img_off[l] = L[l].img_off; fl.lm_off[l] = L[l].lm_off; fl.jac_off[l] = L[l].jac_off;
            }
            size_t dyn = (((size_t)nt_max * ((size_t)nt_max * 12 <= 150 * 1024 ? 12 : 6) + 15) & ~(size_t)15);
            {
                const size_t img_bytes = (size_t)L[levels - 1].w * L[levels - 1].h + 8;
                if (img_bytes <= 150 * 1024) dyn = std::max(dyn, (img_bytes + 15) & ~(size_t)15);
                const size_t both = ((img_bytes + 15) & ~(size_t)15) + (size_t)L[levels - 1].nt * 12;
                if (both <= 150 * 1024) dyn = std::max(dyn, (both + 15) & ~(size_t)15);
            }
            dyn = std::max<size_t>(dyn, 512);
            const bool small_wg = nt_max <= kSmallWgTiles;
            static const int coop_env = []() { const char* e = getenv("VS_GN_HELPERS"); return e ? atoi(e) : -1; }();
            int group = 1;
            if (coop_ok && n_pairs <= kCoopMaxPairs && L[0].nt >= kCoopMinTiles)
                group = coop_env >= 0 ? std::max(1, std::min(coop_env, kCoopMaxGroup)) : std::max(1, std::min(kCoopGroup, cu_count / n_pairs));
            static const int cores_env = []() { const char* e = getenv("VS_GN_CORESIDENT"); return e ? atoi(e) : -1; }();
            const bool cores = small_wg && nt_max <= kCoResidentMaxTiles &&
                    (cores_env >= 0 ? cores_env != 0 : (batch_mode == VS_BATCH_SHARED && n_pairs >= kSharedMinPairs));
            const size_t selbuf_pair = (((size_t)nt_max * 6 + 255) & ~(size_t)255);
            if (cores) {
                group = 1;
                dyn = 16;
                bool need_global = false;
                for (int l = 0; l < levels; l++) {
                    const size_t nt = (size_t)L[l].nt;
                    const size_t need = ((nt <= 32 * (nt256v::kGnThreads / 2) && nt * 12 <= kCoResidentDynMax ? nt * 12 : nt * 6) + 15) & ~(size_t)15;
                    if (need <= kCoResidentDynMax) dyn = std::max(dyn, need); else need_global = true;
                }
                dyn = std::max<size_t>(dyn, 512);
                const size_t want = need_global ? selbuf_pair * (size_t)std::max(cap, n_pairs) : 256;
                if (selbuf_bytes < want) {
                    if (selbuf) (void)hipFree(selbuf);
                    selbuf = nullptr; selbuf_bytes = 0;
                    VS_HIP(vsi::dev_alloc((void**)&selbuf, want));
                    selbuf_bytes = want;
                }
            }
            const auto kernel = cores ? nt256v::vs_k_align_pairs : (small_wg ? nt512::vs_k_align_pairs : nt1024::vs_k_align_pairs);
            const int kthreads = cores ? nt256v::kGnThreads : (small_wg ? nt512::kGnThreads : nt1024::kGnThreads);
            {
                static std::mutex dyn_mu;
                static size_t dyn_set[3][kMaxDevices];
                std::lock_guard<std::mutex> g(dyn_mu);
                size_t& granted = dyn_set[cores ? 2 : (small_wg ? 0 : 1)][std::min(std::max(device, 0), kMaxDevices - 1)];
                if (granted < dyn || device >= kMaxDevices) {
                    VS_HIP(hipFuncSetAttribute((const void*)kernel, hipFuncAttributeMaxDynamicSharedMemorySize, (int)std::max(dyn, granted)));
                    granted = std::max(dyn, granted);
                }
            }
            t_begin(VS_STAGE_GN);
            const int epoch = ++coop_epoch;
            ck.epoch = epoch;
            PairDescPack dpack{};
            if (direct) for (int q = 0; q < n_pairs; q++) dpack.d[q] = hd[q];
            hipLaunchKernelGGL(kernel, dim3(n_pairs * group), dim3(kthreads), dyn, s,
                               direct ? h_states : states, descs, pyr, pyr_frame, lm, lm_frame, jac, jac_frame, recs, recs_pair, nt_max, (int)dyn,
                               fl, gp, group, coop, epoch, wv, dpack, direct ? 1 : 0, cores ? selbuf : nullptr, selbuf_pair);
            VS_HIP(hipGetLastError());
            t_end(1);
            if (!direct) VS_HIP(hipMemcpyAsync(h_states, states, sizeof(PairState) * n_pairs, hipMemcpyDeviceToHost, s));
        }
    }
    ck.open = true;
    return VS_OK;
}

int vs_aligner::chunk_end() {
    if (!ck.open) return set_error(VS_ERR_ARG, "no chunk in flight on this handle");
    ck.open = false;
    hipStream_t s = stream;
    const int n = ck.n, n_pairs = ck.n_pairs, epoch = ck.epoch;
    const vs_aligner_params& p = ck.p;
    vs_transform* out = ck.out; int32_t* status = ck.status; vs_align_info* infos = ck.infos;
    const std::vector<int>& pair_frame = ck.pair_frame;
    const bool direct = ck.direct;
    bool use_host = ck.use_host;
    const GnParams gp = ck.gp;
    const long long seq0 = ck.seq0;
    auto gidx = [&](int i) -> long long { return clip_len > 0 ? (long long)(i % clip_len) : seq0 + i; };
    if (n_pairs > 0) {
        PairDesc* hd = h_descs;
        static const bool poll_done = []() { const char* e = getenv("VS_GN_POLL"); return e ? atoi(e) != 0 : true; }();
        const float phase_scale = (1 << 2) / float(1 << levels);
        auto apply_phase = [&]() -> int {
            hipLaunchKernelGGL(vs_k_phase_apply, dim3((n_pairs + 255) / 256), dim3(256), 0, s, states, pres, pneg, n_pairs,
                               p.phase_correlate_threshold, phase_scale);
            VS_HIP(hipGetLastError());
            return VS_OK;
        };
        const size_t wd_pair = (size_t)2 * nt_max, recs_pair = (size_t)2 * nt_max * 28;
        if (!use_host) {
            if (direct && poll_done && !timing) {
                const auto t0 = std::chrono::steady_clock::now();
                bool all = false;
                while (!all) {
                    all = true;
                    for (int q = 0; q < n_pairs; q++)
                        if (reinterpret_cast<volatile int32_t*>(&h_states[q].pad)[0] != (int32_t)epoch) { all = false; break; }
                    if (!all && std::chrono::steady_clock::now() - t0 > std::chrono::milliseconds(2)) break;
                }
                std::atomic_thread_fence(std::memory_order_acquire);
                if (!all) VS_HIP(hipStreamSynchronize(s));
                else {
                    const hipError_t qe = hipStreamQuery(s);
                    if (qe != hipSuccess && qe != hipErrorNotReady) VS_HIP(qe);
                }
            } else {
                VS_HIP(hipStreamSynchronize(s));
            }
            for (int q = 0; q < n_pairs; q++)
                if (h_states[q].fail_reason >= 100) use_host = true;
            if (use_host) {
                for (int q = 0; q < n_pairs; q++) { memset(&h_states[q], 0, sizeof(PairState)); h_states[q].status = 1; }
                if (direct) VS_HIP(hipMemcpyAsync(descs, hd, sizeof(PairDesc) * n_pairs, hipMemcpyHostToDevice, s));
                VS_HIP(hipMemcpyAsync(states, h_states, sizeof(PairState) * n_pairs, hipMemcpyHostToDevice, s));
                if (p.phase_correlate) VS_TRY(apply_phase());
                VS_HIP(hipStreamSynchronize(s));
            }
        }
        for (int l = levels - 1; use_host && l >= 0; l--) {
            const LevelDims& ld = L[l];
            t_begin(VS_STAGE_WARPDIFF);
            hipLaunchKernelGGL(vs_k_warpdiff_batch, dim3((ld.nt + 255) / 256, n_pairs, 2), dim3(256), 0, s, states, descs, pyr,
                               pyr_frame, ld.img_off, ld.w, ld.h, lm, lm_frame, ld.lm_off, ld.nt, wd, wv, wd_pair);
            VS_HIP(hipGetLastError());
            t_end(1);
            {
                const auto t0 = std::chrono::steady_clock::now();
                VS_HIP(hipMemcpyAsync(h_wd, wd, (size_t)n_pairs * wd_pair * 2, hipMemcpyDeviceToHost, s));
                VS_HIP(hipMemcpyAsync(h_states, states, sizeof(PairState) * n_pairs, hipMemcpyDeviceToHost, s));
                VS_HIP(hipStreamSynchronize(s));
                VS_TRY(select_host(n_pairs, ld));
                VS_HIP(hipMemcpyAsync(idx, h_idx, (size_t)n_pairs * wd_pair * 4, hipMemcpyHostToDevice, s));
                if (timing) tm.ms[VS_STAGE_SELECT] += std::chrono::duration<double, std::milli>(std::chrono::steady_clock::now() - t0).count();
            }
            if (ld.nsel > 0) {
                t_begin(VS_STAGE_GATHER);
                hipLaunchKernelGGL(vs_k_gather_selected, dim3((ld.nsel + 255) / 256, n_pairs, 2), dim3(256), 0, s, states,
                                   descs, pyr, pyr_frame, ld.img_off, ld.w, ld.h, lm, lm_frame, ld.lm_off, jac, jac_frame,
                                   ld.jac_off, ld.nt, ld.nsel, idx, wd_pair, wv, recs, recs_pair, nt_max);
                VS_HIP(hipGetLastError());
                t_end(1);
            }
            t_begin(VS_STAGE_GN);
            if (nt_max <= kSmallWgTiles)
                hipLaunchKernelGGL(nt512::vs_k_gn_level, dim3(n_pairs), dim3(nt512::kGnThreads), 0, s, states, descs, pyr, pyr_frame,
                                   ld.img_off, ld.w, ld.h, ld.nsel, recs, recs_pair, nt_max, l, gp);
            else
                hipLaunchKernelGGL(nt1024::vs_k_gn_level, dim3(n_pairs), dim3(nt1024::kGnThreads), 0, s, states, descs, pyr, pyr_frame,
                                   ld.img_off, ld.w, ld.h, ld.nsel, recs, recs_pair, nt_max, l, gp);
            VS_HIP(hipGetLastError());
            t_end(1);
        }
        if (use_host) {
            VS_HIP(hipMemcpyAsync(h_states, states, sizeof(PairState) * n_pairs, hipMemcpyDeviceToHost, s));
            VS_HIP(hipStreamSynchronize(s));
        }
        for (int q = 0; q < n_pairs; q++) {
            const int i = pair_frame[q];
            const PairState& st = h_states[q];
            vs_align_info& inf = infos[i];
            inf.status = st.status; inf.fail_reason = st.fail_reason; inf.fail_level = st.fail_level;
            for (int l = 0; l < levels; l++) {
                inf.iterations[l] = st.iterations[l]; inf.condition[l] = st.condition[l]; tm.gn_iterations += st.iterations[l];
                if (st.iterations[l] > 0) {
                    inf.selected_x[l] = L[l].nsel; inf.selected_y[l] = L[l].nsel;
                    inf.level_transform[l] = vs_transform{st.level_T[l][0], st.level_T[l][1], st.level_T[l][2], st.level_T[l][3]};
                }
            }
            if (p.phase_correlate) { inf.phase_dx = h_pres[q].dx; inf.phase_dy = h_pres[q].dy; inf.phase_response = h_pres[q].response; }
            vs_transform t{st.T[0], st.T[1], st.T[2], st.T[3]};
            if (st.status == 1) {
                if ((gidx(i) & 1) == 0) t = vs_transform_inverse(&t);
                status[i] = 1;
            }
            out[i] = t;
        }
    } else {
        VS_HIP(hipStreamSynchronize(s));
    }
    if (timing) { t_collect(); tm.frames += n; }
    seq = seq0 + n;
    last_n = n;
    return VS_OK;
}

extern "C" {

static int select_smallest_impl(const uint16_t* warpdiff, int n_arrays, int tx, int ty, float fraction, int32_t* out_idx,
                                int32_t* status, int mem, void* stream, int rule);
int vs_select_smallest(const uint16_t* warpdiff, int n_arrays, int tx, int ty, float fraction, int32_t* out_idx,
                       int32_t* status, int mem, void* stream) try {
    VS_ARG(status);
    return select_smallest_impl(warpdiff, n_arrays, tx, ty, fraction, out_idx, status, mem, stream, 0);
} VS_CATCH_ALL
int vs_select_smallest_stable(const uint16_t* warpdiff, int n_arrays, int tx, int ty, float fraction, int32_t* out_idx, int mem,
                              void* stream) try {
    return select_smallest_impl(warpdiff, n_arrays, tx, ty, fraction, out_idx, nullptr, mem, stream, 1);
} VS_CATCH_ALL
static int select_smallest_impl(const uint16_t* warpdiff, int n_arrays, int tx, int ty, float fraction, int32_t* out_idx,
                                int32_t* status, int mem, void* stream, int rule) {
    VS_ARG(warpdiff && out_idx && (status || rule) && n_arrays >= 1 && tx >= 1 && ty >= 1 && fraction > 0.0f && fraction <= 1.0f);
    const int nt = tx * ty;
    if (nt > kSelectCap) return set_error(VS_ERR_UNSUPPORTED, "%d tiles exceed the on-device selection capacity %d", nt, kSelectCap);
    if (!vsi::device_ready()) return VS_ERR_HIP;
    hipStream_t s = (hipStream_t)stream;
    const int nsel = (int)static_cast<size_t>((size_t)nt * fraction);
    vsi::Staged a, o, st;
    VS_TRY(a.in(warpdiff, (size_t)n_arrays * nt * 2, mem, s));
    VS_TRY(o.out(out_idx, (size_t)n_arrays * nt * 4, mem));
    if (status) VS_TRY(st.out(status, (size_t)n_arrays * 4, mem));
    const size_t dyn = std::max<size_t>((((size_t)nt * 6 + 15) & ~(size_t)15), (((size_t)nt * 4 + 128 + 15) & ~(size_t)15));
    const bool small_wg = nt <= kSmallWgTiles;
    const auto kernel = small_wg ? nt512::vs_k_select : nt1024::vs_k_select;
    VS_HIP(hipFuncSetAttribute((const void*)kernel, hipFuncAttributeMaxDynamicSharedMemorySize, (int)dyn));
    hipLaunchKernelGGL(kernel, dim3(n_arrays), dim3(small_wg ? nt512::kGnThreads : nt1024::kGnThreads), dyn, s, a.as<uint16_t>(), nt,
                       nsel, o.as<int32_t>(), status ? st.as<int32_t>() : (int32_t*)nullptr, rule);
    VS_HIP(hipGetLastError());
    if (status) VS_TRY(vsi::finish_outputs(mem, s, {&o, &st}));
    else VS_TRY(vsi::finish_outputs(mem, s, {&o}));
    return nsel;
}

vs_aligner* vs_aligner_create(const vs_aligner_params* params, int device) try {
    if (!vsi::device_ready()) return nullptr;
    int n = 0;
    if (hipGetDeviceCount(&n) != hipSuccess || device < 0 || device >= n) {
        set_error(VS_ERR_ARG, "device %d out of range (%d devices)", device, n);
        return nullptr;
    }
    if (hipSetDevice(device) != hipSuccess) { set_error(VS_ERR_HIP, "hipSetDevice(%d) failed", device); return nullptr; }
    vs_aligner* a = new vs_aligner();
    a->device = device;
    {
        hipDeviceProp_t prop;
        if (hipGetDeviceProperties(&prop, device) == hipSuccess) {
            if (prop.multiProcessorCount > 0) a->cu_count = prop.multiProcessorCount;
            a->coop_ok = strncmp(prop.gcnArchName, "gfx950", 6) == 0;
        }
    }
    if (params) a->params = *params; else vs_aligner_params_default(&a->params);
    {
        static const int env_mode = []() {
            const char* e = getenv("VS_SELECT_MODE");
            const int m = e ? atoi(e) : -1;
            if (m == VS_SELECT_STL_HOST || m == VS_SELECT_DEVICE || m == VS_SELECT_STABLE) {
                fprintf(stderr, "libvs_amd: VS_SELECT_MODE=%d -- new aligner / stabilizer handles start in selection mode %d (%s)\n", m, m,
                        m == VS_SELECT_STABLE ? "VS_SELECT_STABLE" : (m == VS_SELECT_DEVICE ? "VS_SELECT_DEVICE" : "VS_SELECT_STL_HOST"));
                return m;
            }
            return -1;
        }();
        if (env_mode >= 0) a->select_mode = env_mode;
    }
    const hipError_t se = hipStreamCreateWithFlags(&a->stream, hipStreamNonBlocking);
    if (se != hipSuccess) {
        set_error(VS_ERR_HIP, "hipStreamCreate failed");
        delete a;
        return nullptr;
    }
    return a;
} VS_CATCH_ALL_NULL

void vs_aligner_destroy(vs_aligner* a) {
    if (!a) return;
    (void)hipSetDevice(a->device);
    delete a;
}

int vs_aligner_set_select_mode(vs_aligner* a, int mode) try {
    VS_ARG(a && (mode == VS_SELECT_STL_HOST || mode == VS_SELECT_DEVICE || mode == VS_SELECT_STABLE));
    a->select_mode = mode;
    return VS_OK;
} VS_CATCH_ALL

int vs_aligner_get_select_mode(const vs_aligner* a) try {
    VS_ARG(a);
    return a->select_mode;
} VS_CATCH_ALL

int vs_aligner_set_batch_mode(vs_aligner* a, int mode) try {
    VS_ARG(a && (mode == VS_BATCH_EXCLUSIVE || mode == VS_BATCH_SHARED));
    a->batch_mode = mode;
    return VS_OK;
} VS_CATCH_ALL

int vs_aligner_reset(vs_aligner* a) try {
    VS_ARG(a);
    a->seq = 0;
    return VS_OK;
} VS_CATCH_ALL

void* vs_aligner_stream(const vs_aligner* a) { return a ? (void*)a->stream : nullptr; }

int vs_aligner_wait_stream(vs_aligner* a, void* producer_stream) try {
    VS_ARG(a);
    VS_HIP(hipSetDevice(a->device));
    hipEvent_t ev = nullptr;
    VS_HIP(hipEventCreateWithFlags(&ev, hipEventDisableTiming));
    hipError_t e = hipEventRecord(ev, (hipStream_t)producer_stream);
    if (e == hipSuccess) e = hipStreamWaitEvent(a->stream, ev, 0);
    (void)hipEventDestroy(ev);
    VS_HIP(e);
    return VS_OK;
} VS_CATCH_ALL

}

static int align_start_impl(vs_aligner* a, const void* frames, size_t frame_stride, int n, int w, int h, int stride, int format, int mem,
                            const vs_aligner_params* params, vs_transform* out, int32_t* status, bool async);
static void align_close_clips(vs_aligner* a) {
    if (a->started_clips) { a->started_clips = false; a->clip_len = 0; a->seq = 0; }
}
static void align_failed(vs_aligner* a) {
    a->seq = 0;
    (void)hipStreamSynchronize(a->stream);
    a->ck.open = false;
    for (vs_aligner::Span& sp : a->spans) { a->event_pool.push_back(sp.a); a->event_pool.push_back(sp.b); }
    a->spans.clear();
}
static int align_start(vs_aligner* a, const void* frames, size_t frame_stride, int n, int clip_frames, int w, int h, int stride, int format,
                       int mem, const vs_aligner_params* params, vs_transform* out, int32_t* status, bool async) {
    VS_ARG(a && clip_frames >= 0);
    if (a->started || a->ck.open) return set_error(VS_ERR_ARG, "an alignment is already in flight on this handle");
    a->started_result = 0;
    if (clip_frames > 0) { a->seq = 0; a->clip_len = clip_frames; a->started_clips = true; }
    const int r = vsi::guarded([&] { return align_start_impl(a, frames, frame_stride, n, w, h, stride, format, mem, params, out, status, async); });
    if (r < 0) { a->started = false; align_close_clips(a); if (r != VS_ERR_ARG) align_failed(a); }
    return r;
}
static int align_finish(vs_aligner* a) {
    int r = a->started_result;
    if (a->started) {
        a->started = false;
        r = vsi::guarded([&] { return a->chunk_end(); });
        if (r == VS_OK) for (int i = 0; i < a->started_n; i++) r += a->started_status[i];
    }
// ... 58 lines not shown
            hipError_t e = hipSetDevice(a->device);
            if (e != hipSuccess) return e;
            e = hipMemcpyAsync(a->ingest[c & 1], (const uint8_t*)frames + (size_t)off * step_bytes, (size_t)(m - 1) * step_bytes + frame_bytes,
                               hipMemcpyHostToDevice, a->copy_stream);
            return e != hipSuccess ? e : hipStreamSynchronize(a->copy_stream);
        };
        const int n_chunks = (n + host_chunk - 1) / host_chunk;
        std::future<hipError_t> next = run_async(upload, 0);
        for (int c = 0; c < n_chunks; c++) {
            const int off = c * host_chunk, m = std::min(host_chunk, n - off);
            const hipError_t ue = next.get();
            if (c + 1 < n_chunks) next = run_async(upload, c + 1);
            int r = ue == hipSuccess ? VS_OK : set_error(VS_ERR_HIP, "frame upload failed: %s", hipGetErrorString(ue));
            if (r == VS_OK) r = a->ensure_capacity(m);
            if (r == VS_OK) r = a->run_chunk(a->ingest[c & 1], frame_stride, m, stride, VS_MEM_DEVICE, p, out + off, status + off, a->info.data() + off);
            if (r != VS_OK) { if (next.valid()) (void)next.get(); return r; }
        }
    } else if (async && mem == VS_MEM_DEVICE && n <= max_chunk) {
        VS_TRY(a->ensure_capacity(n));
        VS_TRY(a->chunk_begin(frames, frame_stride, n, stride, mem, p, out, status, a->info.data()));
        a->started = true; a->started_n = n; a->started_status = status;
        return VS_OK;
    } else {
        for (int off = 0; off < n; off += max_chunk) {
            const int m = std::min(max_chunk, n - off);
            VS_TRY(a->ensure_capacity(m));
            const uint8_t* base = (const uint8_t*)frames + (size_t)off * frame_stride * esz;
            VS_TRY(a->run_chunk(base, frame_stride, m, stride, mem, p, out + off, status + off, a->info.data() + off));
        }
    }
    for (int i = 0; i < n; i++) aligned += status[i];
    a->started_result = aligned;
    return VS_OK;
}

extern "C" {

int vs_aligner_align_clips(vs_aligner* a, const void* frames, size_t frame_stride, int n_clips, int frames_per_clip, int w,
                           int h, int stride, int format, int mem, const vs_aligner_params* params, vs_transform* out,
                           int32_t* status) try {
    VS_ARG(a && n_clips >= 1 && frames_per_clip >= 1 && (long long)n_clips * frames_per_clip <= 0x7fffffff);
    const int r = align_start(a, frames, frame_stride, n_clips * frames_per_clip, frames_per_clip, w, h, stride, format, mem, params, out,
                              status, false);
    return r < 0 ? r : align_finish(a);
} VS_CATCH_ALL

int vs_aligner_align_next(vs_aligner* a, const void* frame, int w, int h, int stride, int format, int mem,
                          const vs_aligner_params* params, vs_transform* out) try {
    int32_t st = 0;
    int r = vs_aligner_align_batch(a, frame, 0, 1, w, h, stride, format, mem, params, out, &st);
    if (r < 0) return r;
    return st;
} VS_CATCH_ALL

int vs_aligner_enable_timing(vs_aligner* a, int enable) try {
    VS_ARG(a);
    a->timing = enable != 0;
    memset(&a->tm, 0, sizeof(a->tm));
    return VS_OK;
} VS_CATCH_ALL

int vs_aligner_get_timings(vs_aligner* a, vs_stage_timings* out) try {
    VS_ARG(a && out);
    *out = a->tm;
    return VS_OK;
} VS_CATCH_ALL

int vs_aligner_get_info(const vs_aligner* a, int i, vs_align_info* info) try {
    VS_ARG(a && info && i >= 0 && i < (int)a->info.size());
    *info = a->info[i];
    return VS_OK;
} VS_CATCH_ALL

int vs_aligner_level_dims(const vs_aligner* a, int level, int* w, int* h, int* tx, int* ty, int* ts) try {
    VS_ARG(a && level >= 0 && level < a->levels);
    const LevelDims& l = a->L[level];
    if (w) *w = l.w; if (h) *h = l.h; if (tx) *tx = l.tx; if (ty) *ty = l.ty; if (ts) *ts = l.ts;
    return VS_OK;
} VS_CATCH_ALL

int vs_aligner_read_level_image(const vs_aligner* a, int i, int level, uint8_t* out) try {
    VS_ARG(a && out && level >= 0 && level < a->levels && i >= 0 && i < a->last_n);
    const LevelDims& l = a->L[level];
    VS_HIP(hipSetDevice(a->device));
    VS_HIP(hipMemcpy(out, a->pyr + (size_t)(i + 1) * a->pyr_frame + l.img_off, (size_t)l.w * l.h, hipMemcpyDeviceToHost));
    return VS_OK;
} VS_CATCH_ALL
int vs_aligner_read_level_argmax(const vs_aligner* a, int i, int level, int set, uint16_t* out) try {
    VS_ARG(a && out && level >= 0 && level < a->levels && i >= 0 && i < a->last_n && (set == 0 || set == 1));
    const LevelDims& l = a->L[level];
    VS_HIP(hipSetDevice(a->device));
    std::vector<uint16_t> pairs((size_t)l.nt * 2);
    VS_HIP(hipMemcpy(pairs.data(), a->lm + (size_t)(i + 1) * a->lm_frame + l.lm_off + (size_t)set * 2 * l.nt, (size_t)l.nt * 4,
                     hipMemcpyDeviceToHost));
    for (int t = 0; t < l.nt; t++) { out[t] = pairs[2 * (size_t)t]; out[(size_t)l.nt + t] = pairs[2 * (size_t)t + 1]; }
    return VS_OK;
} VS_CATCH_ALL
int vs_aligner_read_level_jacobian(const vs_aligner* a, int i, int level, int set, float* out) try {
    VS_ARG(a && out && level >= 0 && level < a->levels && i >= 0 && i < a->last_n && (set == 0 || set == 1));
    const LevelDims& l = a->L[level];
    VS_HIP(hipSetDevice(a->device));
    std::vector<float> quads((size_t)l.nt * 4);
    VS_HIP(hipMemcpy(quads.data(), a->jac + (size_t)(i + 1) * a->jac_frame + l.jac_off + (size_t)set * 4 * l.nt, (size_t)l.nt * 16,
                     hipMemcpyDeviceToHost));
    for (int t = 0; t < l.nt; t++)
        for (int c = 0; c < 4; c++) out[(size_t)c * l.nt + t] = quads[4 * (size_t)t + c];
    return VS_OK;
} VS_CATCH_ALL

}

struct vs_stabilizer {
    vs_stabilizer_params params;
    vs_aligner* aligner = nullptr;
    vs_smoother* smoother = nullptr;
    int frame_index = 0;
    std::deque<vs_transform> measurements;
    std::deque<int> meas_ok;
    int border_fill = 0;
    struct SharpBlock { unsigned long long* dev; size_t cap; int refs; };
    std::vector<SharpBlock*> sharp_blocks, sharp_pending;
    int deblur = 0;
    vs_deblur_params deblur_params{2.0f, 4.0f};
    void* deblur_buf = nullptr; size_t deblur_bytes = 0;
    struct Held { void* ptr; bool owned; SharpBlock* sb = nullptr; const unsigned long long* sharp = nullptr; };
    std::deque<Held> frames;
    std::vector<void*> pool;
    size_t frame_bytes = 0;
    void* batch_in = nullptr; size_t batch_in_bytes = 0;
    void* batch_out[2] = {nullptr, nullptr}; size_t batch_out_bytes[2] = {0, 0};
    std::future<hipError_t> down[2];
    hipEvent_t down_ev[2] = {nullptr, nullptr};
    hipStream_t down_stream = nullptr, up_stream = nullptr;
    void* pipe_in[2] = {nullptr, nullptr}; size_t pipe_in_bytes = 0;
    void* span_in[2] = {nullptr, nullptr}; size_t span_in_bytes[2] = {0, 0};
    hipStream_t warp_stream = nullptr;
    hipEvent_t warp_ev = nullptr;
    bool overlap_warps = false;
    bool defer_own = false;
    std::vector<void*> held_release;
    std::vector<vs_transform> t_buf[2];
    std::vector<int32_t> st_buf[2];
    int tb = 0;
    bool prefetched = false;
    const void* next_frames = nullptr; int next_n = 0;
    vs_transform accum{0, 0, 0, 0}, last_meas{0, 0, 0, 0};
    int last_success = 0;
    int w = 0, h = 0, fmt = -1;
};

static void sharp_unhold(vs_stabilizer* s, vs_stabilizer::Held& f) {
    if (f.sb) s->sharp_pending.push_back(f.sb);
    f.sb = nullptr; f.sharp = nullptr;
}
static void sharp_settle(vs_stabilizer* s) {
    for (auto* b : s->sharp_pending) --b->refs;
    s->sharp_pending.clear();
}
static void stab_drop_frames(vs_stabilizer* s) {
    for (auto& f : s->frames) { sharp_unhold(s, f); if (f.owned) (void)hipFree(f.ptr); }
    for (void* p : s->pool) (void)hipFree(p);
    s->frames.clear();
    s->pool.clear();
}

extern "C" {

vs_stabilizer* vs_stabilizer_create(const vs_stabilizer_params* params, int device) try {
// ... 622 lines not shown
```

video_stabilizer_amd/csrc/vs_kernels.hip:

```cpp
#include "vs_kernels.hpp"
#include <cstdlib>
#include <algorithm>

#include <utility>
#include "vs_device.hpp"

using namespace vsd;

namespace {
constexpr int PD_TW = 64, PD_TH = 16;
constexpr int PD_IW = 2 * PD_TW + 8;
constexpr int PD_IH = 2 * PD_TH + 3;
constexpr int PD_IWP = PD_IW;
}

__device__ __forceinline__ void pyr_passes(const uint8_t (*tile)[PD_IWP], uint32_t (*hsum)[PD_TW / 2], int x0, int y0,
                                           uint8_t* __restrict__ out, int ow, int oh, int out_stride) {
    for (int i = threadIdx.x; i < PD_IH * (PD_TW / 2); i += 256) {
        const int r = i >> 5, p = i & 31;
        const uint32_t* row = (const uint32_t*)&tile[r][0];
        const uint32_t d0 = row[p], d1 = row[p + 1], d2 = row[p + 2];
        uint32_t h0 = __builtin_amdgcn_udot4(__builtin_amdgcn_alignbyte(d1, d0, 2), 0x04060401u, 0u, false);
        h0 = __builtin_amdgcn_udot4(d1, 0x00010000u, h0, false);
        uint32_t h1 = __builtin_amdgcn_udot4(d1, 0x04060401u, 0u, false);
// ... 235 lines not shown
                typedef uint32_t u32x3 __attribute__((ext_vector_type(3)));
                const u32x3 t = *(const u32x3*)gp;
                q[0] = t.x; q[1] = t.y; q[2] = t.z;
            } else {
                typedef uint32_t u32x2 __attribute__((ext_vector_type(2)));
                typedef uint32_t u32x4 __attribute__((ext_vector_type(4)));
                const u32x4 ta = *(const u32x4*)gp;
                const u32x2 tb = *(const u32x2*)(gp + 4);
                q[0] = ta.x; q[1] = ta.y; q[2] = ta.z; q[3] = ta.w; q[QW - 2] = tb.x; q[QW - 1] = tb.y;
            }
        };
        auto load_group = [&](uint32_t (&q)[QW], int gy, int gxc) {
            load_group_at(q, (__umul24((uint32_t)gy, (uint32_t)src_stride) + (uint32_t)(gxc * 3)) * (uint32_t)sizeof(T));
        };
        auto border_sel = [&](int gx, int gxc) {
            uint32_t sel = 0;
#pragma unroll
            for (int k = 0; k < 4; k++) sel |= (uint32_t)(clampi(gx + k, 0, w - 1) - gxc) << (8 * k);
            return sel;
        };
        const int r_own = 2 + (tid >> 5), c_own = 1 + (tid & 31);
        const int gx_own = ix0 + 4 * c_own, gxc_own = min(gx_own, w - 4);
        int r_h, c_h;
        if (tid < 3 * 34) { const int k = (tid >= 34) + (tid >= 68); r_h = k == 2 ? PD_IH - 1 : k; c_h = tid - 34 * k; }
        else { const int t = min(tid - 3 * 34, 63); r_h = 2 + (t >> 1); c_h = (t & 1) * 33; }
        const bool has_halo = tid < N_ITEMS - 1024;
        const int gx_h = ix0 + 4 * c_h, gxc_h = clampi(gx_h, 0, w - 4);
        uint32_t q[5][QW];
        uint32_t* const tile_w = (uint32_t*)&tile[0][0];
        const bool interior = g0_aligned && ix0 >= 0 && ix0 + PD_IW <= w && iy0 >= 0 && iy0 + PD_IH <= h;
        if (interior) {
            const uint32_t o_own = (__umul24((uint32_t)(iy0 + r_own), (uint32_t)src_stride) + (uint32_t)(gx_own * 3)) * (uint32_t)sizeof(T);
            const uint32_t o_step = 8u * (uint32_t)src_stride * (uint32_t)sizeof(T);
#pragma unroll
            for (int it = 0; it < 4; it++) load_group_at(q[it], o_own + (uint32_t)it * o_step);
            load_group_at(q[4], (__umul24((uint32_t)(iy0 + r_h), (uint32_t)src_stride) + (uint32_t)(gx_h * 3)) * (uint32_t)sizeof(T));
            const uint32_t g_own = __umul24((uint32_t)(iy0 + r_own), (uint32_t)w) + (uint32_t)gx_own, g_step = 8u * (uint32_t)w;
            const int t_own = r_own * (PD_IWP / 4) + c_own;
#pragma unroll
            for (int it = 0; it < 4; it++) {
                const uint32_t v = gray_word(q[it]);
                tile_w[t_own + 8 * it * (PD_IWP / 4)] = v;
                *(uint32_t*)(g0 + (g_own + (uint32_t)it * g_step)) = v;
            }
            if (has_halo) tile_w[r_h * (PD_IWP / 4) + c_h] = gray_word(q[4]);
        } else {
#pragma unroll
        for (int it = 0; it < 4; it++) load_group(q[it], min(iy0 + r_own + 8 * it, h - 1), gxc_own);
        load_group(q[4], clampi(iy0 + r_h, 0, h - 1), gxc_h);
        const bool own_border = gx_own != gxc_own, own_dword = g0_aligned && gx_own + 3 < w;
        const uint32_t own_sel = border_sel(gx_own, gxc_own);
#pragma unroll
        for (int it = 0; it < 4; it++) {
            uint32_t v = gray_word(q[it]);
            if (own_border) v = __builtin_amdgcn_perm(0u, v, own_sel);
            const int r = r_own + 8 * it, oy = iy0 + r;
            tile_w[r * (PD_IWP / 4) + c_own] = v;
            if (oy < h && gx_own < w) {
                uint8_t* dst = g0 + (__umul24((uint32_t)oy, (uint32_t)w) + (uint32_t)gx_own);
                if (own_dword) *(uint32_t*)dst = v;
                else for (int k = 0; k < 4 && gx_own + k < w; k++) dst[k] = (uint8_t)(v >> (8 * k));
            }
        }
        if (has_halo) {
            uint32_t v = gray_word(q[4]);
            if (gx_h != gxc_h) v = __builtin_amdgcn_perm(0u, v, border_sel(gx_h, gxc_h));
            tile_w[r_h * (PD_IWP / 4) + c_h] = v;
        }
        }
    } else {
        for (int i = threadIdx.x; i < N_ITEMS; i += 256) {
            const int r = i / (PD_IW / 4), c4 = (i - r * (PD_IW / 4)) * 4;
            const int gy = clampi(iy0 + r, 0, h - 1), gx = ix0 + c4;
            const T* row = src + (size_t)gy * src_stride;
            uint32_t v = 0;
#pragma unroll
            for (int k = 0; k < 4; k++) v |= gray_of(row + (size_t)clampi(gx + k, 0, w - 1) * 3, shift_to_8) << (8 * k);
            stage(r, c4, gx, v);
        }
    }
    __syncthreads();
    pyr_passes(tile, hsum, x0, y0, g1, ow, oh, ow);
    }
    }
}

__global__ __launch_bounds__(256) void vs_k_grad_xy(const uint8_t* __restrict__ in, int w, int h, int stride,
                                                    float* __restrict__ gx, float* __restrict__ gy) {
    const int x = blockIdx.x * 256 + threadIdx.x, y = blockIdx.y;
    if (x >= w) return;
    const uint8_t* row = in + (size_t)y * stride;
    float l = (float)row[max(x - 1, 0)], r = (float)row[min(x + 1, w - 1)];
    float u = (float)in[(size_t)max(y - 1, 0) * stride + x], d = (float)in[(size_t)min(y + 1, h - 1) * stride + x];
    gx[(size_t)y * w + x] = 0.5f * (r - l);
    gy[(size_t)y * w + x] = 0.5f * (d - u);
}

__global__ __launch_bounds__(256) void vs_k_grad_argmax(const float* __restrict__ gx, const float* __restrict__ gy,
                                                        int w, int h, int ts, int tx, int ty,
                                                        uint16_t* __restrict__ lmx, uint16_t* __restrict__ lmy) {
    const int tile = blockIdx.x * 4 + (threadIdx.x >> 6), lane = threadIdx.x & 63;
    if (tile >= tx * ty) return;
    const int tyi = tile / tx, txi = tile % tx;
    const int bx = txi * ts, by = tyi * ts, n = ts * ts;
    unsigned long long kx = 0, ky = 0;
    for (int i = lane; i < n; i += 64) {
        int ry = i / ts, rx = i % ts;
        size_t o = (size_t)(by + ry) * w + (bx + rx);
        unsigned long long inv = 0xffffffffu - (unsigned)i;
        unsigned long long a = ((unsigned long long)__float_as_uint(fabsf(gx[o])) << 32) | inv;
        unsigned long long b = ((unsigned long long)__float_as_uint(fabsf(gy[o])) << 32) | inv;
        kx = a > kx ? a : kx;
        ky = b > ky ? b : ky;
    }
    kx = wave_max_u64(kx);
    ky = wave_max_u64(ky);
    if (lane == 0) {
        const size_t nt = (size_t)tx * ty;
        int ix = (int)(0xffffffffu - (unsigned)(kx & 0xffffffffu)), iy = (int)(0xffffffffu - (unsigned)(ky & 0xffffffffu));
        lmx[tile] = (uint16_t)(bx + ix % ts);
        lmx[nt + tile] = (uint16_t)(by + ix / ts);
        lmy[tile] = (uint16_t)(bx + iy % ts);
        lmy[nt + tile] = (uint16_t)(by + iy / ts);
    }
}

__global__ __launch_bounds__(256) void vs_k_sparse_jac(const float* __restrict__ gx, const float* __restrict__ gy,
                                                       int w, int h, const uint16_t* __restrict__ lmx,
                                                       const uint16_t* __restrict__ lmy, int nt,
                                                       float* __restrict__ jx, float* __restrict__ jy) {
    const int i = blockIdx.x * 256 + threadIdx.x;
    if (i >= nt) return;
    const float cx = (float)w * 0.5f, cy = (float)h * 0.5f, scale = 1.f / (float)w;
    int ix0 = min((int)lmx[i], w - 1), iy0 = min((int)lmx[nt + i], h - 1);
    int ix1 = min((int)lmy[i], w - 1), iy1 = min((int)lmy[nt + i], h - 1);
    float u0 = (float)ix0 - cx, v0 = (float)iy0 - cy, u1 = (float)ix1 - cx, v1 = (float)iy1 - cy;
    float g0 = gx[(size_t)iy0 * w + ix0], g1 = gy[(size_t)iy1 * w + ix1];
    jx[i] = 2.f * g0 * u0 * scale;
    jx[nt + i] = 2.f * g0 * (-v0) * scale;
    jx[2 * (size_t)nt + i] = 2.f * g0;
    jx[3 * (size_t)nt + i] = 0.f;
    jy[i] = 2.f * g1 * v1 * scale;
    jy[nt + i] = 2.f * g1 * u1 * scale;
    jy[2 * (size_t)nt + i] = 0.f;
    jy[3 * (size_t)nt + i] = 2.f * g1;
}

__device__ __forceinline__ uint64_t load_u64_unaligned(const uint8_t* p) {
    uint64_t r;
    __builtin_memcpy(&r, p, 8);
    return r;
}

__global__ __launch_bounds__(256) void vs_k_keyframe(const uint8_t* __restrict__ img, int w, int h, int stride,
                                                     int ts, int tx, int ty, uint16_t* __restrict__ lmx,
                                                     uint16_t* __restrict__ lmy, float* __restrict__ jx,
                                                     float* __restrict__ jy, size_t img_frame_stride,
                                                     size_t lm_frame_stride, size_t jac_frame_stride, bool aos) {
    img += blockIdx.y * img_frame_stride;
    lmx += blockIdx.y * lm_frame_stride; lmy += blockIdx.y * lm_frame_stride;
    jx += blockIdx.y * jac_frame_stride; jy += blockIdx.y * jac_frame_stride;
    const int tile = blockIdx.x * 16 + (threadIdx.x >> 4), lane = threadIdx.x & 15;
    const bool live = tile < tx * ty;
    const int tyi = live ? tile / tx : 0, txi = live ? tile % tx : 0;
    const int bx = txi * ts, by = tyi * ts;
    const int chunks = (ts + 7) >> 3, items = live ? ts * chunks : 0;
// ... 395 lines not shown
        return (int)src[(size_t)yy * src_stride + (size_t)xx * channels + c];
    };
    for (int c = 0; c < channels; c++) {
        const int v00 = tap(sx, sy, c), v01 = tap(sx + 1, sy, c), v10 = tap(sx, sy + 1, c), v11 = tap(sx + 1, sy + 1, c);
        int r;
        if (sizeof(T) == 1) {
            r = (v00 * (a0 * b0 * 32) + v01 * (a1 * b0 * 32) + v10 * (a0 * b1 * 32) + v11 * (a1 * b1 * 32) + (1 << 14)) >> 15;
        } else {
            const float k = 1.0f / 1024.0f;
            const float sum = (float)v00 * ((float)(a0 * b0) * k) + (float)v01 * ((float)(a1 * b0) * k) + (float)v10 * ((float)(a0 * b1) * k) +
                              (float)v11 * ((float)(a1 * b1) * k);
            r = (int)rintf(sum);
        }
        dst[(size_t)y * dst_stride + (size_t)x * channels + c] = (T)min(max(r, 0), max_value);
    }
}

__global__ __launch_bounds__(256) void vs_k_calib_copy12(const uint32_t* __restrict__ src, uint32_t* __restrict__ dst,
                                                         size_t n_groups) {
    typedef uint32_t u32x3 __attribute__((ext_vector_type(3)));
    for (size_t i = (size_t)blockIdx.x * 256 + threadIdx.x; i < n_groups; i += (size_t)gridDim.x * 256)
        *(u32x3*)(dst + 3 * i) = *(const u32x3*)(src + 3 * i);
}

namespace vsk {

static inline int cdiv(int a, int b) { return (a + b - 1) / b; }

hipError_t calib_copy12(const void* src, void* dst, size_t bytes, hipStream_t s) {
    hipLaunchKernelGGL(vs_k_calib_copy12, dim3(4096), dim3(256), 0, s, (const uint32_t*)src, (uint32_t*)dst, bytes / 12);
    return hipGetLastError();
}

hipError_t pyr_down(const uint8_t* in, int w, int h, int in_stride, uint8_t* out, int ow, int oh, int out_stride,
                    int n_frames, size_t in_fs, size_t out_fs, hipStream_t s) {
    if (ow <= 0 || oh <= 0 || n_frames <= 0) return hipSuccess;
    const int strips_x = cdiv(ow, 2 * PR_LIVE);
    const int bands = cdiv(oh, n_frames <= 4 ? 4 : PR_OUT);
    const dim3 grid(cdiv(strips_x * bands, 4), n_frames);
#define VS_PD(ROWS, NARROW)                                                                                             \
    hipLaunchKernelGGL((vs_k_pyr_down_rows<ROWS, NARROW>), grid, dim3(256), 0, s, in, w, h, in_stride, out, ow, oh, out_stride, in_fs, \
                       out_fs, strips_x, bands)
    if (n_frames <= 4) { if (w < 4) VS_PD(4, true); else VS_PD(4, false); }
    else { if (w < 4) VS_PD(PR_OUT, true); else VS_PD(PR_OUT, false); }
#undef VS_PD
    return hipGetLastError();
}

hipError_t bgr_to_gray(const void* src, int w, int h, int src_stride, int bits, int shift_to_8, uint8_t* dst,
                       int dst_stride, int n_frames, size_t src_fs, size_t dst_fs, hipStream_t s) {
    dim3 grid(cdiv(w, 1024), h, n_frames);
    if (bits == 8)
        hipLaunchKernelGGL(vs_k_bgr_to_gray<uint8_t>, grid, dim3(256), 0, s, (const uint8_t*)src, w, h, src_stride,
                           shift_to_8, dst, dst_stride, src_fs, dst_fs);
    else
        hipLaunchKernelGGL(vs_k_bgr_to_gray<uint16_t>, grid, dim3(256), 0, s, (const uint16_t*)src, w, h, src_stride,
                           shift_to_8, dst, dst_stride, src_fs, dst_fs);
    return hipGetLastError();
}

hipError_t ingest_pyr(const void* src, int w, int h, int src_stride, int bits, int shift_to_8, uint8_t* g0, uint8_t* g1,
                      int n_frames, size_t src_fs, size_t pyr_fs, hipStream_t s) {
    const int ow = w / 2, oh = h / 2;
    const int tiles_x = cdiv(w, 2 * PD_TW), tiles_y = cdiv(h, 2 * PD_TH);
    const long long tpf = (long long)tiles_x * tiles_y;
    if (tpf > 0x3fffffLL || tiles_x > 1024) return hipErrorNotSupported;
    const int chunk = (int)((tpf + 7) / 8);
    const uint32_t magic = (uint32_t)(0x100000000ULL / (uint32_t)tiles_x) + 1u;
    const size_t esz = bits == 8 ? 1 : 2;
    for (int f0 = 0; f0 < n_frames; f0 += 65535) {
        const int nf = std::min(65535, n_frames - f0);
        const dim3 grid((unsigned)(chunk * 8), (unsigned)nf);
        const uint8_t* sp = (const uint8_t*)src + (size_t)f0 * src_fs * esz;
        if (bits == 8)
            hipLaunchKernelGGL(vs_k_ingest_pyr<uint8_t>, grid, dim3(256), 0, s, (const uint8_t*)sp, w, h, src_stride, shift_to_8,
                               g0 + (size_t)f0 * pyr_fs, g1 + (size_t)f0 * pyr_fs, ow, oh, src_fs, pyr_fs, tiles_x, magic, (int)tpf, chunk);
        else
            hipLaunchKernelGGL(vs_k_ingest_pyr<uint16_t>, grid, dim3(256), 0, s, (const uint16_t*)sp, w, h, src_stride, shift_to_8,
                               g0 + (size_t)f0 * pyr_fs, g1 + (size_t)f0 * pyr_fs, ow, oh, src_fs, pyr_fs, tiles_x, magic, (int)tpf, chunk);
    }
    return hipGetLastError();
}

hipError_t grad_xy(const uint8_t* in, int w, int h, int stride, float* gx, float* gy, hipStream_t s) {
    hipLaunchKernelGGL(vs_k_grad_xy, dim3(cdiv(w, 256), h), dim3(256), 0, s, in, w, h, stride, gx, gy);
    return hipGetLastError();
}

hipError_t grad_argmax(const float* gx, const float* gy, int w, int h, int ts, uint16_t* lmx, uint16_t* lmy,
                       hipStream_t s) {
    int tx = w / ts, ty = h / ts;
    if (tx * ty == 0) return hipSuccess;
    hipLaunchKernelGGL(vs_k_grad_argmax, dim3(cdiv(tx * ty, 4)), dim3(256), 0, s, gx, gy, w, h, ts, tx, ty, lmx, lmy);
    return hipGetLastError();
}

hipError_t sparse_jac(const float* gx, const float* gy, int w, int h, const uint16_t* lmx, const uint16_t* lmy,
                      int nt, float* jx, float* jy, hipStream_t s) {
    if (nt == 0) return hipSuccess;
    hipLaunchKernelGGL(vs_k_sparse_jac, dim3(cdiv(nt, 256)), dim3(256), 0, s, gx, gy, w, h, lmx, lmy, nt, jx, jy);
    return hipGetLastError();
}

hipError_t keyframe(const uint8_t* img, int w, int h, int stride, int ts, uint16_t* lmx, uint16_t* lmy, float* jx,
                    float* jy, int n_frames, size_t img_fs, size_t lm_fs, size_t jac_fs, hipStream_t s, bool aos) {
    int tx = w / ts, ty = h / ts;
    if (tx * ty == 0) return hipSuccess;
#define VS_ROWS(TS)                                                                                                     \
    case TS: {                                                                                                          \
        constexpr int tpw = keyframe_rows_tiles_per_wave(TS);                                                           \
        const int strips_x = cdiv(tx, tpw);                                                                             \
        hipLaunchKernelGGL(vs_k_keyframe_rows<TS>, dim3(cdiv(strips_x * ty, 4), n_frames), dim3(256), 0, s, img, w, h,  \
                           stride, tx, ty, lmx, lmy, jx, jy, img_fs, lm_fs, jac_fs, strips_x, aos);                     \
        break;                                                                                                          \
    }
    switch (ts) {
        VS_ROWS(2) VS_ROWS(4) VS_ROWS(6) VS_ROWS(8) VS_ROWS(10) VS_ROWS(12) VS_ROWS(14) VS_ROWS(16) VS_ROWS(18) VS_ROWS(20)
    default:
        hipLaunchKernelGGL(vs_k_keyframe, dim3(cdiv(tx * ty, 16), n_frames), dim3(256), 0, s, img, w, h, stride, ts, tx, ty,
                           lmx, lmy, jx, jy, img_fs, lm_fs, jac_fs, aos);
    }
#undef VS_ROWS
    return hipGetLastError();
}

bool keyframe_levels_supported(const KeyframeLevels& L) {
    for (int i = 0; i < L.n; i++)
        if (L.lv[i].ts < 2 || L.lv[i].ts > 20 || (L.lv[i].ts & 1) || L.lv[i].tx * L.lv[i].ty == 0) return false;
    return L.n >= 1 && L.n <= 16;
}
hipError_t keyframe_levels(const uint8_t* pyr, uint16_t* lm, float* jac, KeyframeLevels L, int n_frames, size_t pyr_fs, size_t lm_fs,
                           size_t jac_fs, hipStream_t s) {
    int total = 0;
    for (int i = 0; i < L.n; i++) {
        const int ts = L.lv[i].ts, tpw = keyframe_rows_tiles_per_wave(ts);
        L.lv[i].strips_x = cdiv(L.lv[i].tx, tpw);
        L.lv[i].blocks = cdiv(L.lv[i].strips_x * L.lv[i].ty, 4);
        total += L.lv[i].blocks;
    }
    hipLaunchKernelGGL(vs_k_keyframe_levels, dim3(total, n_frames), dim3(256), 0, s, pyr, lm, jac, pyr_fs, lm_fs, jac_fs, L);
    return hipGetLastError();
}

hipError_t sparse_warpdiff(const uint8_t* tmpl, const uint8_t* key, int w, int h, int stride, const uint16_t* lm,
                           int nt, float A, float B, float TX, float TY, uint16_t* out, hipStream_t s) {
    if (nt == 0) return hipSuccess;
    hipLaunchKernelGGL(vs_k_sparse_warpdiff, dim3(cdiv(nt, 256)), dim3(256), 0, s, tmpl, key, w, h, stride, lm, nt, A, B,
                       TX, TY, out);
    return hipGetLastError();
}

hipError_t sparse_ica(const uint8_t* tmpl, const uint8_t* key, int w, int h, int stride, const uint16_t* selx, int nx,
                      const uint16_t* sely, int ny, const float* jacx, const float* jacy, float A, float B, float TX,
                      float TY, double* out, hipStream_t s) {
    hipLaunchKernelGGL(vs_k_sparse_ica, dim3(1), dim3(1024), 0, s, tmpl, key, w, h, stride, selx, nx, sely, ny, jacx,
                       jacy, A, B, TX, TY, out);
    return hipGetLastError();
}

hipError_t image_warp(const uint8_t* in, int w, int h, int stride, float A, float B, float TX, float TY, float* out,
                      int ow, int oh, hipStream_t s) {
    hipLaunchKernelGGL(vs_k_image_warp, dim3(cdiv(ow, 256), oh), dim3(256), 0, s, in, w, h, stride, A, B, TX, TY, out, ow,
                       oh);
    return hipGetLastError();
}

// ... 46 lines not shown
```

video_stabilizer_amd/csrc/vs_kernels.hpp:

```cpp
#pragma once

#include <hip/hip_runtime.h>
#include <stddef.h>
#include <stdint.h>

namespace vsk {

struct Roi { int x, y, w, h; };

hipError_t calib_copy12(const void* src, void* dst, size_t bytes, hipStream_t s);

hipError_t pyr_down(const uint8_t* in, int w, int h, int in_stride, uint8_t* out, int ow, int oh, int out_stride,
                    int n_frames, size_t in_frame_stride, size_t out_frame_stride, hipStream_t s);
hipError_t bgr_to_gray(const void* src, int w, int h, int src_stride, int bits, int shift_to_8, uint8_t* dst,
                       int dst_stride, int n_frames, size_t src_frame_stride, size_t dst_frame_stride, hipStream_t s);
hipError_t ingest_pyr(const void* src, int w, int h, int src_stride, int bits, int shift_to_8, uint8_t* g0, uint8_t* g1,
                      int n_frames, size_t src_frame_stride, size_t pyr_frame_stride, hipStream_t s);
hipError_t grad_xy(const uint8_t* in, int w, int h, int stride, float* gx, float* gy, hipStream_t s);
hipError_t grad_argmax(const float* gx, const float* gy, int w, int h, int ts, uint16_t* lmx, uint16_t* lmy,
                       hipStream_t s);
hipError_t sparse_jac(const float* gx, const float* gy, int w, int h, const uint16_t* lmx, const uint16_t* lmy, int nt,
                      float* jx, float* jy, hipStream_t s);
hipError_t keyframe(const uint8_t* img, int w, int h, int stride, int ts, uint16_t* lmx, uint16_t* lmy, float* jx,
                    float* jy, int n_frames, size_t img_frame_stride, size_t lm_frame_stride, size_t jac_frame_stride,
                    hipStream_t s, bool aos = false);
struct KeyframeLevel { int w, h, ts, tx, ty, strips_x, blocks; size_t img_off, lm_off, jac_off; };
struct KeyframeLevels { int n; KeyframeLevel lv[16]; };
bool keyframe_levels_supported(const KeyframeLevels& L);
hipError_t keyframe_levels(const uint8_t* pyr, uint16_t* lm, float* jac, KeyframeLevels L, int n_frames, size_t pyr_frame_stride,
                           size_t lm_frame_stride, size_t jac_frame_stride, hipStream_t s);
hipError_t sparse_warpdiff(const uint8_t* tmpl, const uint8_t* key, int w, int h, int stride, const uint16_t* lm,
                           int nt, float A, float B, float TX, float TY, uint16_t* out, hipStream_t s);
hipError_t sparse_ica(const uint8_t* tmpl, const uint8_t* key, int w, int h, int stride, const uint16_t* selx, int nx,
                      const uint16_t* sely, int ny, const float* jacx, const float* jacy, float A, float B, float TX,
                      float TY, double* out, hipStream_t s);
hipError_t image_warp(const uint8_t* in, int w, int h, int stride, float A, float B, float TX, float TY, float* out,
                      int ow, int oh, hipStream_t s);
hipError_t bgr_warp_generic(const void* src, int w, int h, int src_stride, int channels, int bits,
                            const float4* params_dev, int mode, int border, int max_value, void* dst, int dst_stride,
                            bool f32out, int n_frames, size_t src_frame_stride, size_t dst_frame_stride, Roi roi, hipStream_t s);
hipError_t bgr_warp_c3(const void* src, int w, int h, int src_stride, int bits, const float4* params_dev, const float4* extents_dev,
                       int mode, int border, int max_value, void* dst, int dst_stride, int n_frames, size_t src_fs, size_t dst_fs, Roi roi,
                       int compact, hipStream_t s);
int bgr_warp_c3_compact_shape(const float* E4, int n_frames);
hipError_t bgr_warp_cv_generic(const void* src, int w, int h, int src_stride, int channels, int bits, const double* minv_dev, int border,
                               int max_value, void* dst, int dst_stride, int n_frames, size_t src_fs, size_t dst_fs, Roi roi, hipStream_t s);
size_t bgr_warp_cv_table_ints(int bits, Roi roi);
constexpr int kCvInlineFrames = 64;
hipError_t bgr_warp_cv_c3(const void* src, int w, int h, int src_stride, int bits, const double* minv_dev, const double* minv_host, int* tab_dev, int border, int max_value,
                          void* dst, int dst_stride, int n_frames, size_t src_fs, size_t dst_fs, Roi roi, hipStream_t s);
struct FillCand { double m[6]; const void* src; unsigned long long reserved; };
hipError_t bgr_warp_cv_fill_c3(const FillCand* cands_dev, int n_cand, int w, int h, int src_stride, int bits, int max_value, void* dst, int dst_stride,
                               int n_frames, size_t dst_fs, Roi roi, hipStream_t s);
struct DeblurCand { double m[6]; const void* src; const unsigned long long* sharp; };
hipError_t bgr_sharpness(const void* src, int w, int h, int src_stride, int bits, int shift_to_8, unsigned long long* out, int n_frames, size_t src_fs,
                         hipStream_t s);
hipError_t bgr_deblur(const DeblurCand* cands_dev, float* r2_dev, int n_cand, int w, int h, int src_stride, int bits, int shift_to_8, int max_value,
                      float sensitivity, float max_ratio, void* dst, int dst_stride, int n_frames, size_t dst_fs, bool targets_aligned, hipStream_t s);
void bgr_warp_c3_extents(const float* P4, int n_frames, Roi roi, int bits, int mode, float* E4);

}
```

Before: 85020.

## Gather template pixels into per-pair sparse tables instead of dense template pyramids

Adds a template_table kernel that, for each pair, samples template intensities only at the keypoint locations and stores them in a compact per-pair table. For color inputs without phase correlation, it avoids building full dense pyramids for even-indexed template frames, computing gray and Gaussian-downsampled values directly from the source frame at keypoints. The warp-diff, gather and fused GN kernels then read the compact table instead of the full pyramid. The cost is an extra kernel launch and a per-pair table allocation, plus redundant per-point 5x5 and deeper-window filtering at the coarse levels.

```diff
diff --git a/include/vs_amd.h b/include/vs_amd.h
--- a/include/vs_amd.h
+++ b/include/vs_amd.h
@@ -196,6 +196,7 @@
 int  vs_aligner_get_info(const vs_aligner* a, int i, vs_align_info* info);
 int  vs_aligner_level_dims(const vs_aligner* a, int level, int* w, int* h, int* tiles_x, int* tiles_y, int* tile_size);
 int  vs_aligner_read_level_image(const vs_aligner* a, int i, int level, uint8_t* out);
+int  vs_aligner_read_template_pixels(const vs_aligner* a, int pair, int level, int set, uint8_t* out);
 int  vs_aligner_read_level_argmax(const vs_aligner* a, int i, int level, int set, uint16_t* out);
 int  vs_aligner_read_level_jacobian(const vs_aligner* a, int i, int level, int set, float* out);
 
diff --git a/video_stabilizer_amd/capi.py b/video_stabilizer_amd/capi.py
--- a/video_stabilizer_amd/capi.py
+++ b/video_stabilizer_amd/capi.py
@@ -161,6 +161,7 @@
     "vs_aligner_get_info": (_i32, [_vp, _i32, C.POINTER(AlignInfo)]),
     "vs_aligner_level_dims": (_i32, [_vp, _i32, _IP, _IP, _IP, _IP, _IP]),
     "vs_aligner_read_level_image": (_i32, [_vp, _i32, _i32, _vp]),
+    "vs_aligner_read_template_pixels": (_i32, [_vp, _i32, _i32, _i32, _vp]),
     "vs_aligner_read_level_argmax": (_i32, [_vp, _i32, _i32, _i32, _vp]),
     "vs_aligner_read_level_jacobian": (_i32, [_vp, _i32, _i32, _i32, _vp]),
     "vs_stabilizer_create": (_vp, [C.POINTER(StabilizerParams), _i32]),
@@ -779,6 +780,16 @@
         d["img"] = img
         return d
 
+    def template_pixels(self, pair, level):
+        tx, ty = (C.c_int() for _ in range(2))
+        _check(lib().vs_aligner_level_dims(self.h, level, None, None, C.byref(tx), C.byref(ty), None))
+        out = []
+        for s in (0, 1):
+            tp = np.empty((ty.value, tx.value), np.uint8)
+            _check(lib().vs_aligner_read_template_pixels(self.h, pair, level, s, _p(tp)))
+            out.append(tp)
+        return out
+
     def keyframe_tables(self, i, level):
         w, h, tx, ty, ts = (C.c_int() for _ in range(5))
         _check(lib().vs_aligner_level_dims(self.h, level, *(C.byref(v) for v in (w, h, tx, ty, ts))))
diff --git a/video_stabilizer_amd/csrc/vs_align_kernels.inc b/video_stabilizer_amd/csrc/vs_align_kernels.inc
--- a/video_stabilizer_amd/csrc/vs_align_kernels.inc
+++ b/video_stabilizer_amd/csrc/vs_align_kernels.inc
@@ -1006,7 +1006,8 @@
                                                                int nt_cap, int dyn_bytes, FusedLevels fl, GnParams gp,
                                                                int group, uint8_t* __restrict__ coop, int epoch,
                                                                float* __restrict__ wv_all, PairDescPack dpack, int direct,
-                                                               uint8_t* __restrict__ selbuf, size_t selbuf_pair) {
+                                                               uint8_t* __restrict__ selbuf, size_t selbuf_pair,
+                                                               const uint8_t* __restrict__ tpx, size_t tpx_pair) {
     extern __shared__ __attribute__((aligned(16))) uint8_t dyn[];
     __shared__ SelShared ss2[2];
     __shared__ GnShared sh;
@@ -1061,7 +1062,7 @@
             __syncthreads();
             if (my_slice < 0) continue;
         }
-        const uint8_t* tmpl = pyr + (size_t)d.tmpl_slot * pyr_frame + fl.img_off[l];
+        const uint8_t* tmpl = tpx + (size_t)p * tpx_pair + fl.tab_off[l];
         const uint8_t* key = pyr + (size_t)d.key_slot * pyr_frame + fl.img_off[l];
         const PointRecs rc = pair_recs(recs, recs_pair, p, nt_cap);
         float P[4];
@@ -1129,6 +1130,7 @@
             while (base < count) {
                 LanczosFetch f[kWdFlight];
                 uint32_t tp[kWdFlight];
+                int po[kWdFlight];
 #pragma unroll
                 for (int u = 0; u < kWdFlight; u++) {
                     const int tile_x = min((int)lx[u], w - 1), tile_y = min((int)ly[u], h - 1);
@@ -1136,7 +1138,11 @@
                     const float Wx = A1 * ox - P[1] * oy + P[2];
                     const float Wy = P[1] * ox + A1 * oy + P[3];
                     f[u] = lanczos_fetch(gkey, w, h, w, Wx, Wy);
-                    tp[u] = gtmpl[(size_t)tile_y * w + tile_x];
+                    const int i = min(base + u * kGnThreads, count - 1);
+                    int set = 0, t = i;
+                    if (both) point_tile(i, set, t);
+                    po[u] = set * nt + t;
+                    tp[u] = gtmpl[voff + po[u]];
                 }
                 const int nb = base + kWdFlight * kGnThreads;
                 if (nb < count) load_lm(nb);
@@ -1147,9 +1153,7 @@
                     float diff = fabsf(v - (float)tp[u]);
                     diff = fminf(fmaxf(diff, 0.0f), 65535.0f);
                     if (i < count) {
-                        int set = 0, t = i;
-                        if (both) point_tile(i, set, t);
-                        const int o = set * nt + t;
+                        const int o = po[u], t = o >= nt ? o - nt : o;
                         VS_BOUNDS_CHECK(o, both ? 2 * nt : nt, 121);
                         VS_BOUNDS_CHECK(voff + o, 2 * nt_cap, 122);
                         dst[o] = ((uint32_t)(uint16_t)diff << 16) | (uint32_t)t;
@@ -1183,7 +1187,7 @@
                     const int tile_x = min((int)lx[u], w - 1), tile_y = min((int)ly[u], h - 1);
                     const float ox = (float)tile_x, oy = (float)tile_y;
                     f[u] = lanczos_fetch(gkey, w, h, w, A1 * ox - P[1] * oy + P[2], P[1] * ox + A1 * oy + P[3]);
-                    tp[u] = gtmpl[(size_t)tile_y * w + tile_x];
+                    tp[u] = gtmpl[i0 + min(base + u * kGnThreads, n - 1)];
                 }
 #pragma unroll
                 for (int u = 0; u < 4; u++) {
diff --git a/video_stabilizer_amd/csrc/vs_engine.hip b/video_stabilizer_amd/csrc/vs_engine.hip
--- a/video_stabilizer_amd/csrc/vs_engine.hip
+++ b/video_stabilizer_amd/csrc/vs_engine.hip
@@ -4,6 +4,7 @@
 #include "vs_device.hpp"
 
 #include <algorithm>
+#include <array>
 #include <atomic>
 #include <chrono>
 #include <mutex>
@@ -45,13 +46,11 @@
     double level_T[kMaxLevels][4];
 };
 
-struct PairDesc {
-    int32_t tmpl_slot;
-    int32_t key_slot;
-};
+typedef vsk::PairSlots PairDesc;
 
 constexpr int kDirectMaxPairs = 16;
-struct PairDescPack { PairDesc d[kDirectMaxPairs]; };
+typedef vsk::PairSlotsPack PairDescPack;
+static_assert(sizeof(PairDescPack) == kDirectMaxPairs * sizeof(PairDesc), "the pack holds kDirectMaxPairs descriptors");
 
 struct GnParams {
     double threshold, max_displacement;
@@ -81,14 +80,15 @@
                                                            size_t img_off, int w, int h,
                                                            const uint16_t* __restrict__ lm_tab, size_t lm_frame,
                                                            size_t lm_off, int nt, uint16_t* __restrict__ wd,
-                                                           float* __restrict__ wv, size_t wd_pair) {
+                                                           float* __restrict__ wv, size_t wd_pair,
+                                                           const uint8_t* __restrict__ tpx, size_t tpx_pair, int tab_off) {
     const int p = blockIdx.y, set = blockIdx.z;
     const PairState& st = states[p];
     if (st.status != 1) return;
     const int i = blockIdx.x * 256 + threadIdx.x;
     if (i >= nt) return;
     const PairDesc d = descs[p];
-    const uint8_t* tmpl = pyr + (size_t)d.tmpl_slot * pyr_frame + img_off;
+    const uint8_t* tmpl = tpx + (size_t)p * tpx_pair + tab_off + (size_t)set * nt;
     const uint8_t* key = pyr + (size_t)d.key_slot * pyr_frame + img_off;
     const uint16_t* lm = lm_tab + (size_t)d.key_slot * lm_frame + lm_off + (size_t)set * 2 * nt;
     double T[4] = {st.T[0], st.T[1], st.T[2], st.T[3]};
@@ -100,7 +100,7 @@
     float Wx = (1.0f + P[0]) * ox - P[1] * oy + P[2];
     float Wy = P[1] * ox + (1.0f + P[0]) * oy + P[3];
     float v = lanczos_sample_u8(key, w, h, w, Wx, Wy);
-    float diff = fabsf(v - (float)tmpl[(size_t)tile_y * w + tile_x]);
+    float diff = fabsf(v - (float)tmpl[i]);
     diff = fminf(fmaxf(diff, 0.0f), 65535.0f);
     wd[(size_t)p * wd_pair + (size_t)set * nt + i] = (uint16_t)diff;
     wv[(size_t)p * wd_pair + (size_t)set * nt + i] = v;
@@ -129,12 +129,11 @@
     return r;
 }
 __device__ __forceinline__ void write_rec(const PointRecs& rc, int slot, const uint16_t* __restrict__ lm,
-                                          const float* __restrict__ jac, int nt, int t, const uint8_t* __restrict__ tmpl,
-                                          int w, int h, const float* __restrict__ wv_set) {
+                                          const float* __restrict__ jac, int nt, int t, const uint8_t* __restrict__ tmpl_set,
+                                          const float* __restrict__ wv_set) {
     const uint32_t xy = ((const uint32_t*)lm)[t];
-    const int px = (int)(xy & 0xffffu), py = (int)(xy >> 16);
     rc.xy[slot] = xy;
-    const float tv = (float)tmpl[(size_t)min(py, h - 1) * w + min(px, w - 1)];
+    const float tv = (float)tmpl_set[t];
     rc.tv[slot] = tv;
     rc.r0[slot] = tv - wv_set[t];
     rc.j[slot] = ((const float4*)jac)[t];
@@ -142,8 +141,7 @@
 
 __global__ __launch_bounds__(256) void vs_k_gather_selected(const PairState* __restrict__ states,
                                                             const PairDesc* __restrict__ descs,
-                                                            const uint8_t* __restrict__ pyr, size_t pyr_frame,
-                                                            size_t img_off, int w, int h,
+                                                            const uint8_t* __restrict__ tpx, size_t tpx_pair, int tab_off,
                                                             const uint16_t* __restrict__ lm_tab, size_t lm_frame,
                                                             size_t lm_off, const float* __restrict__ jac_tab,
                                                             size_t jac_frame, size_t jac_off, int nt, int nsel,
@@ -157,9 +155,9 @@
     const PairDesc d = descs[p];
     const uint16_t* lm = lm_tab + (size_t)d.key_slot * lm_frame + lm_off + (size_t)set * 2 * nt;
     const float* jac = jac_tab + (size_t)d.key_slot * jac_frame + jac_off + (size_t)set * 4 * nt;
-    const uint8_t* tmpl = pyr + (size_t)d.tmpl_slot * pyr_frame + img_off;
+    const uint8_t* tmpl = tpx + (size_t)p * tpx_pair + tab_off + (size_t)set * nt;
     const int t = idx[(size_t)p * idx_pair + (size_t)set * nt + j];
-    write_rec(pair_recs(recs, recs_pair, p, nt_cap), set * nsel + j, lm, jac, nt, t, tmpl, w, h, wv + (size_t)p * idx_pair + (size_t)set * nt);
+    write_rec(pair_recs(recs, recs_pair, p, nt_cap), set * nsel + j, lm, jac, nt, t, tmpl, wv + (size_t)p * idx_pair + (size_t)set * nt);
 }
 
 constexpr int kMaxDevices = 64;
@@ -187,6 +185,7 @@
     int levels;
     int w[kMaxLevels], h[kMaxLevels], nt[kMaxLevels], nsel[kMaxLevels], tx[kMaxLevels];
     unsigned long long img_off[kMaxLevels], lm_off[kMaxLevels], jac_off[kMaxLevels];
+    int tab_off[kMaxLevels];
 };
 
 namespace nt1024 {
@@ -261,6 +260,10 @@
     int32_t* idx = nullptr;
     uint8_t* recs = nullptr;
     uint8_t* coop = nullptr;
+    uint8_t* tpx = nullptr; size_t tpx_pair = 0;
+    vsk::TemplateLevels TL{};
+    bool sparse_templates = true;
+    std::vector<uint8_t> slot_dense;
     uint8_t* selbuf = nullptr; size_t selbuf_bytes = 0;
     int coop_epoch = 0;
     void* stage = nullptr; size_t stage_bytes = 0;
@@ -380,14 +383,14 @@
 
 void vs_aligner::release() {
     release_phase();
-    void* d[] = {pyr, lm, jac, states, descs, wd, wv, idx, recs, coop, stage, ingest[0], ingest[1], selbuf};
+    void* d[] = {pyr, lm, jac, states, descs, wd, wv, idx, recs, coop, stage, ingest[0], ingest[1], selbuf, tpx};
     for (void* p : d) if (p) (void)hipFree(p);
     selbuf = nullptr; selbuf_bytes = 0;
     ingest[0] = ingest[1] = nullptr; ingest_bytes = 0;
     void* hp[] = {h_wd, h_idx, h_states, h_descs};
     for (void* p : hp) if (p) (void)hipHostFree(p);
     pyr = nullptr; lm = nullptr; jac = nullptr; states = nullptr; descs = nullptr; wd = nullptr; wv = nullptr; idx = nullptr;
-    recs = nullptr; coop = nullptr; stage = nullptr; stage_bytes = 0; h_wd = nullptr; h_idx = nullptr; h_states = nullptr; h_descs = nullptr;
+    tpx = nullptr; recs = nullptr; coop = nullptr; stage = nullptr; stage_bytes = 0; h_wd = nullptr; h_idx = nullptr; h_states = nullptr; h_descs = nullptr;
     cap = 0;
 }
 
@@ -423,6 +426,10 @@
         nt_max = std::max(nt_max, l.nt);
     }
     pyr_frame = img; lm_frame = (lmo + 63) & ~(size_t)63; jac_frame = (jo + 63) & ~(size_t)63;
+    TL = vsk::TemplateLevels{};
+    TL.levels = lv; TL.w = w; TL.h = h;
+    for (int i = 0; i < lv; i++) { TL.lv[i].nt = L[i].nt; TL.lv[i].img_off = L[i].img_off; TL.lv[i].lm_off = L[i].lm_off; }
+    tpx_pair = vsk::template_table_layout(TL);
     return VS_OK;
 }
 
@@ -432,22 +439,22 @@
     const size_t slots = (size_t)newcap + 1;
     const size_t coop_bytes = std::min(newcap, kCoopMaxPairs) * coop_pair_bytes(nt_max);
     struct NewSet {
-        void* dev[10] = {};
+        void* dev[11] = {};
         void* pinned[4] = {};
         ~NewSet() {
             for (void* q : dev) if (q) (void)hipFree(q);
             for (void* q : pinned) if (q) (void)hipHostFree(q);
         }
     } ns;
-    enum { D_PYR, D_LM, D_JAC, D_STATES, D_DESCS, D_WD, D_IDX, D_WV, D_RECS, D_COOP };
-    const size_t dev_bytes[10] = {
+    enum { D_PYR, D_LM, D_JAC, D_STATES, D_DESCS, D_WD, D_IDX, D_WV, D_RECS, D_COOP, D_TPX };
+    const size_t dev_bytes[11] = {
         slots * pyr_frame, slots * lm_frame * 2, slots * jac_frame * 4, sizeof(PairState) * newcap, sizeof(PairDesc) * newcap,
         (size_t)newcap * 2 * nt_max * sizeof(uint16_t), (size_t)newcap * 2 * nt_max * sizeof(int32_t),
         (size_t)newcap * 2 * nt_max * sizeof(float) * 2,
-        (size_t)newcap * 2 * nt_max * 28, coop_bytes};
+        (size_t)newcap * 2 * nt_max * 28, coop_bytes, (size_t)newcap * tpx_pair};
     const size_t pinned_bytes[4] = {(size_t)newcap * 2 * nt_max * sizeof(uint16_t), (size_t)newcap * 2 * nt_max * sizeof(int32_t),
                                     sizeof(PairState) * newcap, sizeof(PairDesc) * newcap};
-    for (int i = 0; i < 10; i++) VS_HIP(vsi::dev_alloc(&ns.dev[i], dev_bytes[i]));
+    for (int i = 0; i < 11; i++) VS_HIP(vsi::dev_alloc(&ns.dev[i], dev_bytes[i]));
     for (int i = 0; i < 4; i++) VS_HIP(vsi::pinned_alloc(&ns.pinned[i], pinned_bytes[i]));
     VS_HIP(hipMemsetAsync(ns.dev[D_COOP], 0, coop_bytes, stream));
     const bool carry = pyr && seq > 0;
@@ -457,10 +464,10 @@
         VS_HIP(hipMemcpyAsync(ns.dev[D_JAC], jac + (size_t)last_n * jac_frame, jac_frame * 4, hipMemcpyDeviceToDevice, stream));
     }
     VS_HIP(hipStreamSynchronize(stream));
-    void** dev_members[10] = {(void**)&pyr, (void**)&lm, (void**)&jac, (void**)&states, (void**)&descs, (void**)&wd, (void**)&idx,
-                              (void**)&wv, (void**)&recs, (void**)&coop};
+    void** dev_members[11] = {(void**)&pyr, (void**)&lm, (void**)&jac, (void**)&states, (void**)&descs, (void**)&wd, (void**)&idx,
+                              (void**)&wv, (void**)&recs, (void**)&coop, (void**)&tpx};
     void** pinned_members[4] = {(void**)&h_wd, (void**)&h_idx, (void**)&h_states, (void**)&h_descs};
-    for (int i = 0; i < 10; i++) std::swap(*dev_members[i], ns.dev[i]);
+    for (int i = 0; i < 11; i++) std::swap(*dev_members[i], ns.dev[i]);
     for (int i = 0; i < 4; i++) std::swap(*pinned_members[i], ns.pinned[i]);
     if (carry) last_n = 0;
     coop_epoch = 0;
@@ -535,6 +542,28 @@
         VS_HIP(hipMemcpyAsync(jac, jac + (size_t)last_n * jac_frame, jac_frame * 4, hipMemcpyDeviceToDevice, s));
     }
 
+    auto gidx = [&](int i) -> long long { return clip_len > 0 ? (long long)(i % clip_len) : seq + i; };
+    std::vector<std::pair<int, int>> runs;
+    if (clip_len > 0 && (clip_len & 1)) for (int c0 = 0; c0 < n; c0 += clip_len) runs.emplace_back(c0, std::min(clip_len, n - c0));
+    else runs.emplace_back(0, n);
+    auto odd_of = [&](const std::pair<int, int>& r, int& first_odd, int& n_odd) {
+        first_odd = r.first + ((gidx(r.first) & 1) ? 0 : 1);
+        n_odd = first_odd < r.first + r.second ? (r.first + r.second - first_odd + 1) / 2 : 0;
+    };
+    const bool sparse = sparse_templates && fmt != VS_FMT_GRAY8 && !p.phase_correlate && levels <= 4;
+    slot_dense.assign((size_t)n + 1, 1);
+    std::vector<std::array<int, 3>> dense_runs;
+    if (!sparse) dense_runs.push_back({0, n, 1});
+    else {
+        for (int i = 0; i + 1 < n; i++) if (!(gidx(i) & 1)) slot_dense[(size_t)i + 1] = 0;
+        for (auto& r : runs) {
+            int first_odd, n_odd;
+            odd_of(r, first_odd, n_odd);
+            if (n_odd > 0) dense_runs.push_back({first_odd, n_odd, 2});
+        }
+        if (!(gidx(n - 1) & 1)) dense_runs.push_back({n - 1, 1, 1});
+    }
+
     const void* dframes = frames;
     t_begin(VS_STAGE_INGEST);
     if (mem == VS_MEM_HOST) {
@@ -554,15 +583,20 @@
             VS_HIP(hipMemcpy2DAsync(slot1 + (size_t)i * pyr_frame, W, (const uint8_t*)dframes + (size_t)i * frame_stride,
                                     stride, W, H, hipMemcpyDeviceToDevice, s));
     } else {
-        VS_HIP(vsk::ingest_pyr(dframes, W, H, stride, fbits > 8 ? 16 : 8, fbits - 8, slot1,
-                               slot1 + L[1].img_off, n, frame_stride, pyr_frame, s));
-    }
-    t_end(1);
+        for (auto& r : dense_runs)
+            VS_HIP(vsk::ingest_pyr((const uint8_t*)dframes + (size_t)r[0] * frame_stride * esz, W, H, stride, fbits > 8 ? 16 : 8, fbits - 8,
+                                   slot1 + (size_t)r[0] * pyr_frame, slot1 + (size_t)r[0] * pyr_frame + L[1].img_off, r[1],
+                                   (size_t)r[2] * frame_stride, (size_t)r[2] * pyr_frame, s));
+    }
+    t_end(fmt == VS_FMT_GRAY8 ? 1 : (int)dense_runs.size());
     t_begin(VS_STAGE_PYR_DOWN);
-    for (int l = (fmt == VS_FMT_GRAY8 ? 1 : 2); l < levels; l++)
-        VS_HIP(vsk::pyr_down(slot1 + L[l - 1].img_off, L[l - 1].w, L[l - 1].h, L[l - 1].w, slot1 + L[l].img_off, L[l].w,
-                             L[l].h, L[l].w, n, pyr_frame, pyr_frame, s));
-    t_end(levels - (fmt == VS_FMT_GRAY8 ? 1 : 2));
+    for (auto& r : dense_runs)
+        for (int l = (fmt == VS_FMT_GRAY8 ? 1 : 2); l < levels; l++) {
+            uint8_t* f0 = slot1 + (size_t)r[0] * pyr_frame;
+            VS_HIP(vsk::pyr_down(f0 + L[l - 1].img_off, L[l - 1].w, L[l - 1].h, L[l - 1].w, f0 + L[l].img_off, L[l].w,
+                                 L[l].h, L[l].w, r[1], (size_t)r[2] * pyr_frame, (size_t)r[2] * pyr_frame, s));
+        }
+    t_end((levels - (fmt == VS_FMT_GRAY8 ? 1 : 2)) * (int)dense_runs.size());
 
     if (p.phase_correlate) {
         VS_TRY(ensure_phase());
@@ -573,16 +607,12 @@
         t_end(2);
     }
 
-    auto gidx = [&](int i) -> long long { return clip_len > 0 ? (long long)(i % clip_len) : seq + i; };
     {
-        std::vector<std::pair<int, int>> runs;
-        if (clip_len > 0 && (clip_len & 1)) for (int c0 = 0; c0 < n; c0 += clip_len) runs.emplace_back(c0, std::min(clip_len, n - c0));
-        else runs.emplace_back(0, n);
         bool any = false;
         int kf_launches = 0;
         for (auto& r : runs) {
-            const int first_odd = r.first + ((gidx(r.first) & 1) ? 0 : 1);
-            const int n_odd = first_odd < r.first + r.second ? (r.first + r.second - first_odd + 1) / 2 : 0;
+            int first_odd, n_odd;
+            odd_of(r, first_odd, n_odd);
             if (n_odd <= 0) continue;
             if (!any) { t_begin(VS_STAGE_KEYFRAME); any = true; }
             const size_t so = (size_t)(first_odd + 1);
@@ -627,6 +657,7 @@
             const int cur = i + 1, prev = i;
             if (gidx(i) & 1) { hd[q].key_slot = cur; hd[q].tmpl_slot = prev; }
             else { hd[q].key_slot = prev; hd[q].tmpl_slot = cur; }
+            hd[q].tmpl_frame = slot_dense[(size_t)hd[q].tmpl_slot] ? -1 : hd[q].tmpl_slot - 1;
         }
         for (int q = 0; q < n_pairs; q++) {
             memset(&h_states[q], 0, sizeof(PairState));
@@ -638,6 +669,12 @@
             VS_HIP(hipMemcpyAsync(descs, hd, sizeof(PairDesc) * n_pairs, hipMemcpyHostToDevice, s));
             VS_HIP(hipMemcpyAsync(states, h_states, sizeof(PairState) * n_pairs, hipMemcpyHostToDevice, s));
         }
+        PairDescPack dpack{};
+        if (direct) for (int q = 0; q < n_pairs; q++) dpack.d[q] = hd[q];
+        t_begin(VS_STAGE_INGEST);
+        VS_HIP(vsk::template_table(dframes, stride, frame_stride, fbits > 8 ? 16 : 8, fbits - 8, pyr, pyr_frame, lm, lm_frame, descs,
+                                   direct ? &dpack : nullptr, n_pairs, sparse, tpx, tpx_pair, TL, s));
+        t_end(1);
         std::vector<vsp::Pair> hp;
         std::vector<uint8_t> hneg;
         const float phase_scale = (1 << 2) / float(1 << levels);
@@ -679,7 +716,7 @@
             fl.levels = levels;
             for (int l = 0; l < levels; l++) {
                 fl.w[l] = L[l].w; fl.h[l] = L[l].h; fl.nt[l] = L[l].nt; fl.nsel[l] = L[l].nsel; fl.tx[l] = L[l].tx;
-                fl.img_off[l] = L[l].img_off; fl.lm_off[l] = L[l].lm_off; fl.jac_off[l] = L[l].jac_off;
+                fl.img_off[l] = L[l].img_off; fl.lm_off[l] = L[l].lm_off; fl.jac_off[l] = L[l].jac_off; fl.tab_off[l] = TL.lv[l].tab_off;
             }
             size_t dyn = (((size_t)nt_max * ((size_t)nt_max * 12 <= 150 * 1024 ? 12 : 6) + 15) & ~(size_t)15);
             {
@@ -731,11 +768,9 @@
             t_begin(VS_STAGE_GN);
             const int epoch = ++coop_epoch;
             ck.epoch = epoch;
-            PairDescPack dpack{};
-            if (direct) for (int q = 0; q < n_pairs; q++) dpack.d[q] = hd[q];
             hipLaunchKernelGGL(kernel, dim3(n_pairs * group), dim3(kthreads), dyn, s,
                                direct ? h_states : states, descs, pyr, pyr_frame, lm, lm_frame, jac, jac_frame, recs, recs_pair, nt_max, (int)dyn,
-                               fl, gp, group, coop, epoch, wv, dpack, direct ? 1 : 0, cores ? selbuf : nullptr, selbuf_pair);
+                               fl, gp, group, coop, epoch, wv, dpack, direct ? 1 : 0, cores ? selbuf : nullptr, selbuf_pair, tpx, tpx_pair);
             VS_HIP(hipGetLastError());
             t_end(1);
             if (!direct) VS_HIP(hipMemcpyAsync(h_states, states, sizeof(PairState) * n_pairs, hipMemcpyDeviceToHost, s));
@@ -802,7 +837,7 @@
             const LevelDims& ld = L[l];
             t_begin(VS_STAGE_WARPDIFF);
             hipLaunchKernelGGL(vs_k_warpdiff_batch, dim3((ld.nt + 255) / 256, n_pairs, 2), dim3(256), 0, s, states, descs, pyr,
-                               pyr_frame, ld.img_off, ld.w, ld.h, lm, lm_frame, ld.lm_off, ld.nt, wd, wv, wd_pair);
+                               pyr_frame, ld.img_off, ld.w, ld.h, lm, lm_frame, ld.lm_off, ld.nt, wd, wv, wd_pair, tpx, tpx_pair, TL.lv[l].tab_off);
             VS_HIP(hipGetLastError());
             t_end(1);
             {
@@ -817,7 +852,7 @@
             if (ld.nsel > 0) {
                 t_begin(VS_STAGE_GATHER);
                 hipLaunchKernelGGL(vs_k_gather_selected, dim3((ld.nsel + 255) / 256, n_pairs, 2), dim3(256), 0, s, states,
-                                   descs, pyr, pyr_frame, ld.img_off, ld.w, ld.h, lm, lm_frame, ld.lm_off, jac, jac_frame,
+                                   descs, tpx, tpx_pair, TL.lv[l].tab_off, lm, lm_frame, ld.lm_off, jac, jac_frame,
                                    ld.jac_off, ld.nt, ld.nsel, idx, wd_pair, wv, recs, recs_pair, nt_max);
                 VS_HIP(hipGetLastError());
                 t_end(1);
@@ -933,6 +968,10 @@
         }();
         if (env_mode >= 0) a->select_mode = env_mode;
     }
+    {
+        const char* e = getenv("VS_SPARSE_TEMPLATES");
+        a->sparse_templates = !(e && atoi(e) == 0 && e[0] != '\0');
+    }
     const hipError_t se = hipStreamCreateWithFlags(&a->stream, hipStreamNonBlocking);
     if (se != hipSuccess) {
         set_error(VS_ERR_HIP, "hipStreamCreate failed");
@@ -1157,8 +1196,17 @@
 int vs_aligner_read_level_image(const vs_aligner* a, int i, int level, uint8_t* out) try {
     VS_ARG(a && out && level >= 0 && level < a->levels && i >= 0 && i < a->last_n);
     const LevelDims& l = a->L[level];
+    if ((size_t)i + 1 < a->slot_dense.size() && !a->slot_dense[(size_t)i + 1])
+        return set_error(VS_ERR_UNSUPPORTED, "frame %d was only ever a template: it has no dense pyramid (VS_SPARSE_TEMPLATES=0 keeps one for every frame)", i);
     VS_HIP(hipSetDevice(a->device));
     VS_HIP(hipMemcpy(out, a->pyr + (size_t)(i + 1) * a->pyr_frame + l.img_off, (size_t)l.w * l.h, hipMemcpyDeviceToHost));
+    return VS_OK;
+} VS_CATCH_ALL
+int vs_aligner_read_template_pixels(const vs_aligner* a, int pair, int level, int set, uint8_t* out) try {
+    VS_ARG(a && out && level >= 0 && level < a->levels && pair >= 0 && pair < a->ck.n_pairs && a->tpx && (set == 0 || set == 1));
+    const LevelDims& l = a->L[level];
+    VS_HIP(hipSetDevice(a->device));
+    VS_HIP(hipMemcpy(out, a->tpx + (size_t)pair * a->tpx_pair + a->TL.lv[level].tab_off + (size_t)set * l.nt, (size_t)l.nt, hipMemcpyDeviceToHost));
     return VS_OK;
 } VS_CATCH_ALL
 int vs_aligner_read_level_argmax(const vs_aligner* a, int i, int level, int set, uint16_t* out) try {
diff --git a/video_stabilizer_amd/csrc/vs_kernels.hip b/video_stabilizer_amd/csrc/vs_kernels.hip
--- a/video_stabilizer_amd/csrc/vs_kernels.hip
+++ b/video_stabilizer_amd/csrc/vs_kernels.hip
@@ -341,6 +341,183 @@
     __syncthreads();
     pyr_passes(tile, hsum, x0, y0, g1, ow, oh, ow);
     }
+    }
+}
+
+namespace {
+__device__ __forceinline__ uint32_t tpl_down5(const uint8_t* win, int pitch, int r0, int c0) {
+    constexpr uint32_t kTplWeights[5] = {1, 4, 6, 4, 1};
+    uint32_t acc = 0;
+#pragma unroll
+    for (int j = 0; j < 5; j++) {
+        const uint8_t* row = win + (r0 + j) * pitch + c0;
+        acc += kTplWeights[j] * ((uint32_t)row[0] + 4u * row[1] + 6u * row[2] + 4u * row[3] + (uint32_t)row[4]);
+    }
+    return acc >> 8;
+}
+
+template <typename T, int NPX>
+__device__ __forceinline__ void tpl_row_grays(const T* __restrict__ p, int shift_to_8, uint32_t (&g)[NPX]) {
+    constexpr int NB = NPX * 3 * (int)sizeof(T), C = NB >= 16 ? 16 : 8, NFULL = NB / C, NCH = NFULL + (NB % C ? 1 : 0);
+    static_assert(NB >= 8, "rows of at least 8 bytes");
+    uint32_t ch[NCH][C / 4];
+#pragma unroll
+    for (int c = 0; c < NCH; c++) __builtin_memcpy(ch[c], (const uint8_t*)p + (c < NFULL ? c * C : NB - C), C);
+    auto elem = [&](int e) -> uint32_t {
+        const int bo = e * (int)sizeof(T);
+        const int c = bo + (int)sizeof(T) <= NFULL * C ? bo / C : NCH - 1;
+        const int j = bo - (c < NFULL ? c * C : NB - C);
+        return (ch[c][j / 4] >> (8 * (j % 4))) & (sizeof(T) == 1 ? 0xffu : 0xffffu);
+    };
+#pragma unroll
+    for (int k = 0; k < NPX; k++) {
+        uint32_t v = (elem(3 * k) * 3735u + elem(3 * k + 1) * 19235u + elem(3 * k + 2) * 9798u + 16384u) >> 15;
+        v >>= shift_to_8;
+        g[k] = v > 255u ? 255u : v;
+    }
+}
+
+template <int LV> struct TplWin { static constexpr int side0 = (1 << (LV + 2)) - 3; };
+template <typename T, int G, int LV>
+__device__ __forceinline__ uint32_t tpl_point_deep(uint8_t* win, const T* __restrict__ src, int w, int h, int src_stride,
+                                                   int shift_to_8, int x, int y, int lane) {
+    constexpr int S0 = TplWin<LV>::side0;
+    const int o0x = (x << LV) - (S0 - 1) / 2, o0y = (y << LV) - (S0 - 1) / 2;
+    static_assert(S0 <= G, "a lane per window row");
+    if (lane < S0) {
+        const T* __restrict__ row = src + (size_t)clampi(o0y + lane, 0, h - 1) * src_stride;
+        uint8_t* wrow = win + lane * S0;
+        if (o0x >= 0 && o0x + S0 <= w) {
+            uint32_t g[S0];
+            tpl_row_grays<T, S0>(row + (size_t)o0x * 3, shift_to_8, g);
+#pragma unroll
+            for (int c = 0; c < S0; c++) wrow[c] = (uint8_t)g[c];
+        } else {
+            for (int c = 0; c < S0; c++) wrow[c] = (uint8_t)gray_of(row + (size_t)clampi(o0x + c, 0, w - 1) * 3, shift_to_8);
+        }
+    }
+    __syncthreads();
+    uint8_t* prev = win;
+    int sp = S0;
+#pragma unroll
+    for (int k = 1; k < LV; k++) {
+        const int sk = (sp - 3) / 2;
+        const int okx = (x << (LV - k)) - (sk - 1) / 2, oky = (y << (LV - k)) - (sk - 1) / 2;
+        const int wk = w >> k, hk = h >> k;
+        uint8_t* cur = prev + sp * sp;
+        for (int i = lane; i < sk * sk; i += G) {
+            const int cy = i / sk, cx = i - cy * sk;
+            const int vx = clampi(okx + cx, 0, wk - 1), vy = clampi(oky + cy, 0, hk - 1);
+            cur[i] = (uint8_t)tpl_down5(prev, sp, 2 * (vy - oky), 2 * (vx - okx));
+        }
+        __syncthreads();
+        prev = cur;
+        sp = sk;
+    }
+    return tpl_down5(prev, 5, 0, 0);
+}
+template <int LV> constexpr int tpl_win_bytes() {
+    int n = 0;
+    for (int s = TplWin<LV>::side0; s >= 5; s = (s - 3) / 2) n += s * s;
+    return (n + 15) & ~15;
+}
+constexpr int kTplG2 = 16, kTplG3 = 64;
+constexpr int kTplLds = tpl_win_bytes<2>() * (256 / kTplG2) > tpl_win_bytes<3>() * (256 / kTplG3) ? tpl_win_bytes<2>() * (256 / kTplG2)
+                                                                                                  : tpl_win_bytes<3>() * (256 / kTplG3);
+}
+
+template <typename T>
+__global__ __launch_bounds__(256) void vs_k_template_table(const T* __restrict__ src_all, int src_stride, size_t src_frame_stride,
+                                                           int shift_to_8, const uint8_t* __restrict__ pyr, size_t pyr_frame,
+                                                           const uint16_t* __restrict__ lm_tab, size_t lm_frame,
+                                                           const vsk::PairSlots* __restrict__ pairs, vsk::PairSlotsPack pack, int direct,
+                                                           uint8_t* __restrict__ tab, size_t tab_pair, vsk::TemplateLevels A) {
+    __shared__ __attribute__((aligned(16))) uint8_t lds[kTplLds];
+    const int p = blockIdx.y;
+    const vsk::PairSlots d = direct ? pack.d[p] : pairs[p];
+    const bool sparse = d.tmpl_frame >= 0;
+    const T* __restrict__ src = src_all + (size_t)max(d.tmpl_frame, 0) * src_frame_stride;
+    const uint8_t* __restrict__ dense = pyr + (size_t)d.tmpl_slot * pyr_frame;
+    const uint16_t* __restrict__ lm = lm_tab + (size_t)d.key_slot * lm_frame;
+    uint8_t* __restrict__ out = tab + (size_t)p * tab_pair;
+    const int w = A.w, h = A.h;
+    auto keypoint = [&](int l, int j, int& x, int& y) {
+        const uint32_t xy = ((const uint32_t*)(lm + A.lv[l].lm_off))[j];
+        x = min((int)(xy & 0xffffu), (w >> l) - 1);
+        y = min((int)(xy >> 16), (h >> l) - 1);
+    };
+    int b = blockIdx.x;
+    if (b < A.blocks_flat) {
+        const int g = b * 256 + (int)threadIdx.x;
+        if (g >= A.total) return;
+        int l = 0;
+        while (l + 1 < A.levels && g >= A.lv[l + 1].tab_off) l++;
+        if (sparse && l >= 2) return;
+        const int j = g - A.lv[l].tab_off;
+        int x, y;
+        keypoint(l, j, x, y);
+        uint32_t v;
+        if (!sparse) {
+            v = dense[A.lv[l].img_off + (size_t)y * (w >> l) + x];
+        } else if (l == 0) {
+            const T* px = src + (size_t)y * src_stride + (size_t)x * 3;
+            uint32_t a, b;
+            if (sizeof(T) == 1) {
+                const int back = x == w - 1 && y == h - 1 ? 1 : 0;
+                __builtin_memcpy(&a, (const uint8_t*)px - back, 4);
+                a >>= 8 * back;
+                v = ((a & 255u) * 3735u + ((a >> 8) & 255u) * 19235u + ((a >> 16) & 255u) * 9798u + 16384u) >> 15;
+            } else {
+                __builtin_memcpy(&a, px, 4);
+                __builtin_memcpy(&b, px + 1, 4);
+                v = ((a & 0xffffu) * 3735u + (a >> 16) * 19235u + (b >> 16) * 9798u + 16384u) >> 15;
+            }
+            v >>= shift_to_8;
+            v = v > 255u ? 255u : v;
+        } else {
+            constexpr uint32_t kTplWeights[5] = {1, 4, 6, 4, 1};
+            uint32_t acc = 0;
+            if (2 * x - 2 >= 0 && 2 * x + 3 <= w) {
+#pragma unroll
+                for (int jj = 0; jj < 5; jj++) {
+                    uint32_t g[5];
+                    tpl_row_grays<T, 5>(src + (size_t)clampi(2 * y - 2 + jj, 0, h - 1) * src_stride + (size_t)(2 * x - 2) * 3, shift_to_8, g);
+                    acc += kTplWeights[jj] * (g[0] + 4u * g[1] + 6u * g[2] + 4u * g[3] + g[4]);
+                }
+            } else {
+                for (int jj = 0; jj < 5; jj++) {
+                    const T* row = src + (size_t)clampi(2 * y - 2 + jj, 0, h - 1) * src_stride;
+                    uint32_t r = 0;
+#pragma unroll
+                    for (int ii = 0; ii < 5; ii++)
+                        r += kTplWeights[ii] * gray_of(row + (size_t)clampi(2 * x - 2 + ii, 0, w - 1) * 3, shift_to_8);
+                    acc += kTplWeights[jj] * r;
+                }
+            }
+            v = acc >> 8;
+        }
+        out[g] = (uint8_t)v;
+        return;
+    }
+    if (!sparse) return;
+    b -= A.blocks_flat;
+    if (b < A.blocks_l2) {
+        const int n = 2 * A.lv[2].nt, jq = b * (256 / kTplG2) + (int)(threadIdx.x / kTplG2), j = min(jq, n - 1);
+        int x, y;
+        keypoint(2, j, x, y);
+        const uint32_t v = tpl_point_deep<T, kTplG2, 2>(lds + (threadIdx.x / kTplG2) * tpl_win_bytes<2>(), src, w, h, src_stride, shift_to_8,
+                                                        x, y, (int)(threadIdx.x % kTplG2));
+        if (threadIdx.x % kTplG2 == 0 && jq < n) out[A.lv[2].tab_off + j] = (uint8_t)v;
+        return;
+    }
+    b -= A.blocks_l2;
+    {
+        const int n = 2 * A.lv[3].nt, jq = b * (256 / kTplG3) + (int)(threadIdx.x / kTplG3), j = min(jq, n - 1);
+        int x, y;
+        keypoint(3, j, x, y);
+        const uint32_t v = tpl_point_deep<T, kTplG3, 3>(lds + (threadIdx.x / kTplG3) * tpl_win_bytes<3>(), src, w, h, src_stride, shift_to_8,
+                                                        x, y, (int)(threadIdx.x % kTplG3));
+        if (threadIdx.x % kTplG3 == 0 && jq < n) out[A.lv[3].tab_off + j] = (uint8_t)v;
     }
 }
 
@@ -902,6 +1079,36 @@
     return hipGetLastError();
 }
 
+size_t template_table_layout(TemplateLevels& L) {
+    int off = 0;
+    for (int l = 0; l < L.levels; l++) { L.lv[l].tab_off = off; off += 2 * L.lv[l].nt; }
+    L.total = off;
+    return ((size_t)off + 15) & ~(size_t)15;
+}
+
+hipError_t template_table(const void* src, int src_stride, size_t src_fs, int bits, int shift_to_8, const uint8_t* pyr, size_t pyr_fs,
+                          const uint16_t* lm, size_t lm_fs, const PairSlots* pairs, const PairSlotsPack* pack, int n_pairs,
+                          bool any_sparse, uint8_t* tab, size_t tab_pair, TemplateLevels L, hipStream_t s) {
+    if (n_pairs <= 0) return hipSuccess;
+    if (any_sparse && (L.levels > 4 || L.levels < 3)) return hipErrorNotSupported;
+    if (pack && n_pairs > 16) return hipErrorInvalidValue;
+    L.blocks_flat = cdiv(L.total, 256);
+    L.blocks_l2 = any_sparse ? cdiv(2 * L.lv[2].nt, 256 / kTplG2) : 0;
+    L.blocks_l3 = any_sparse && L.levels > 3 ? cdiv(2 * L.lv[3].nt, 256 / kTplG3) : 0;
+    const PairSlotsPack none{};
+    const size_t esz = bits == 8 ? 1 : 2;
+    for (int p0 = 0; p0 < n_pairs; p0 += 65535) {
+        const dim3 grid((unsigned)(L.blocks_flat + L.blocks_l2 + L.blocks_l3), (unsigned)std::min(65535, n_pairs - p0));
+        if (esz == 1)
+            hipLaunchKernelGGL(vs_k_template_table<uint8_t>, grid, dim3(256), 0, s, (const uint8_t*)src, src_stride, src_fs, shift_to_8, pyr,
+                               pyr_fs, lm, lm_fs, pairs ? pairs + p0 : nullptr, pack ? *pack : none, pack ? 1 : 0, tab + (size_t)p0 * tab_pair, tab_pair, L);
+        else
+            hipLaunchKernelGGL(vs_k_template_table<uint16_t>, grid, dim3(256), 0, s, (const uint16_t*)src, src_stride, src_fs, shift_to_8, pyr,
+                               pyr_fs, lm, lm_fs, pairs ? pairs + p0 : nullptr, pack ? *pack : none, pack ? 1 : 0, tab + (size_t)p0 * tab_pair, tab_pair, L);
+    }
+    return hipGetLastError();
+}
+
 hipError_t grad_xy(const uint8_t* in, int w, int h, int stride, float* gx, float* gy, hipStream_t s) {
     hipLaunchKernelGGL(vs_k_grad_xy, dim3(cdiv(w, 256), h), dim3(256), 0, s, in, w, h, stride, gx, gy);
     return hipGetLastError();
diff --git a/video_stabilizer_amd/csrc/vs_kernels.hpp b/video_stabilizer_amd/csrc/vs_kernels.hpp
--- a/video_stabilizer_amd/csrc/vs_kernels.hpp
+++ b/video_stabilizer_amd/csrc/vs_kernels.hpp
@@ -16,6 +16,15 @@
                        int dst_stride, int n_frames, size_t src_frame_stride, size_t dst_frame_stride, hipStream_t s);
 hipError_t ingest_pyr(const void* src, int w, int h, int src_stride, int bits, int shift_to_8, uint8_t* g0, uint8_t* g1,
                       int n_frames, size_t src_frame_stride, size_t pyr_frame_stride, hipStream_t s);
+struct PairSlots { int32_t tmpl_slot, key_slot, tmpl_frame; };
+struct PairSlotsPack { PairSlots d[16]; };
+struct TemplateLevel { int nt, tab_off; size_t img_off, lm_off; };
+struct TemplateLevels { int levels, w, h, total, blocks_flat, blocks_l2, blocks_l3; TemplateLevel lv[16]; };
+size_t template_table_layout(TemplateLevels& L);
+hipError_t template_table(const void* src, int src_stride, size_t src_frame_stride, int bits, int shift_to_8, const uint8_t* pyr,
+                          size_t pyr_frame_stride, const uint16_t* lm, size_t lm_frame_stride, const PairSlots* pairs,
+                          const PairSlotsPack* pack, int n_pairs, bool any_sparse, uint8_t* tab, size_t tab_pair, TemplateLevels L,
+                          hipStream_t s);
 hipError_t grad_xy(const uint8_t* in, int w, int h, int stride, float* gx, float* gy, hipStream_t s);
 hipError_t grad_argmax(const float* gx, const float* gy, int w, int h, int ts, uint16_t* lmx, uint16_t* lmy,
                        hipStream_t s);
```

Result: no change. 84970, median of 2 (-0.1%).
